# NVIDIA/retinanet-examples

Measured on AMD Instinct MI355X. Metric: images/sec end-to-end (incl. decode+NMS), RN50FPN 800px bs=8, higher is better.
Workload: dtype bf16; 1 GPU; ResNet50FPN bf16 inference, bs=8 per GPU at 800x1280, HIP decode x5 + NMS; global_batch=8, parallelism=replicas x1 (no data-path collective), entry=Model.forward (eval), postproc=fused

## Files before the change

### include/odtk_conv.h

```cpp
#ifndef ODTK_CONV_H
#define ODTK_CONV_H

#include <stddef.h>

#ifdef __cplusplus
extern "C" {
#endif

int odtk_conv_bias_act(void *y, const void *x, const void *w, const void *bias, int batch_size, int c_in, int height, int width,
                       int c_out, int kernel_h, int kernel_w, int stride_h, int stride_w, int pad_h, int pad_w, int dtype,
                       int relu, void *stream);

int odtk_conv_bias_act_pads(void *y, const void *x, const void *w, const void *bias, int batch_size, int c_in, int height, int width,
                            int c_out, int kernel_h, int kernel_w, int stride_h, int stride_w, int pad_h, int pad_w, int pad_h_end,
                            int pad_w_end, int dtype, int relu, void *stream);

const char *odtk_conv_last_plan(void);

size_t odtk_conv_plan_export(char *text, size_t capacity);
int odtk_conv_plan_import(const char *text);


int odtk_conv_instance_count(int dtype);

#ifdef __cplusplus
}
#endif
#endif
```

### include/odtk_hip.h

```cpp
#ifndef ODTK_HIP_H
#define ODTK_HIP_H

#include <stddef.h>
#include <stdint.h>

#ifdef __cplusplus
extern "C" {
#endif

#define ODTK_OK                0
#define ODTK_ERR_INVALID      -1
#define ODTK_ERR_WORKSPACE    -2
#define ODTK_ERR_HIP          -3
#define ODTK_ERR_UNSUPPORTED  -4

#define ODTK_MAX_LEVELS    6
#define ODTK_MAX_ANCHORS   32
#define ODTK_MAX_TOP_N     16384
#define ODTK_MAX_NMS_COUNT 7680
#define ODTK_MAX_NMS_COUNT_SCRATCH (1 << 22)
#define ODTK_MAX_NMS_DETECTIONS 2048

#define ODTK_F32   0
#define ODTK_BF16  1
#define ODTK_F16   2

#define ODTK_FLAG_ROTATED        1u
#define ODTK_FLAG_LOGITS         2u
#define ODTK_FLAG_ROTATED_NMS_FIXED_ANGLE 4u

const char *odtk_version(void);
int odtk_abi_struct_size(int which);
const char *odtk_last_hip_error(void);

int odtk_decode(int batch_size, const void *const *inputs, void *const *outputs,
                size_t height, size_t width, size_t scale, size_t num_anchors, size_t num_classes,
                const float *anchors, size_t anchors_len, float score_thresh, int top_n,
                void *workspace, size_t workspace_size, void *stream);

int odtk_decode_rotate(int batch_size, const void *const *inputs, void *const *outputs,
                       size_t height, size_t width, size_t scale, size_t num_anchors, size_t num_classes,
                       const float *anchors, size_t anchors_len, float score_thresh, int top_n,
                       void *workspace, size_t workspace_size, void *stream);

int odtk_nms(int batch_size, const void *const *inputs, void *const *outputs,
             size_t count, int detections_per_im, float nms_thresh,
             void *workspace, size_t workspace_size, void *stream);

int odtk_nms_rotate(int batch_size, const void *const *inputs, void *const *outputs,
                    size_t count, int detections_per_im, float nms_thresh,
                    void *workspace, size_t workspace_size, void *stream);

int odtk_iou(const void *const *inputs, void *const *outputs, int num_boxes, int num_anchors,
             void *stream);


typedef struct odtk_level {
  const void *cls;
  const void *box;
  int32_t height, width;
  int32_t stride;
  int32_t channels_last;
  const float *anchors;
  const float *cls_bias;
  const float *box_bias;
  const float *cls_thresholds;
} odtk_level_t;

#define ODTK_THRESHOLD_TABLE_FLOATS(channels) ((size_t)(channels) + 8)
int odtk_prefilter_thresholds(const float *cls_bias, int channels, int dtype, float score_thresh, float *table, void *stream);

int odtk_decode_levels(int batch_size, int n_levels, const odtk_level_t *levels,
                       int num_anchors, int num_classes, int dtype, uint32_t flags,
                       float score_thresh, int top_n,
                       void *const *outputs, int n_outputs,
                       void *workspace, size_t workspace_size, void *stream);

int odtk_nms_ex(int batch_size, const void *const *inputs, void *const *outputs, int n_outputs,
                size_t count, int detections_per_im, float nms_thresh, uint32_t flags,
                void *workspace, size_t workspace_size, void *stream);

int odtk_nms_sorted_runs(int batch_size, const void *const *inputs, void *const *outputs, int n_outputs, size_t count,
                         int run_len, const uint32_t *run_valid, int detections_per_im, float nms_thresh, uint32_t flags,
                         void *workspace, size_t workspace_size, void *stream);

int odtk_detect(int batch_size, int n_levels, const odtk_level_t *levels,
                int num_anchors, int num_classes, int dtype, uint32_t flags,
                float score_thresh, int top_n, float nms_thresh, int detections_per_im,
                void *const *outputs, void *workspace, size_t workspace_size, void *stream);

int odtk_bias_act(void *y, const float *bias, const void *residual, size_t n_pixels, int channels,
                  int dtype, int relu, void *stream);

int odtk_bias_act_maxpool(const void *y, const float *bias, void *out, int batch_size, int height, int width,
                          int channels, int dtype, int relu, void *stream);

int odtk_upsample_nearest2x(const void *x, void *out, int batch_size, int height, int width, int channels, int dtype,
                            void *stream);

int odtk_stem_pack(const void *x, void *out, int batch_size, int height, int width, int in_dtype, int channels_last, int out_dtype,
                   void *stream);

typedef struct odtk_image {
  uint64_t src_offset;
  int32_t src_width, src_height, src_pitch;
  int32_t out_width, out_height;
  int32_t mirror;
  int32_t x_table, y_table;
  int32_t x_taps, y_taps;
} odtk_image_t;
int odtk_preprocess_images(int batch_size, const odtk_image_t *images, const void *src, size_t src_bytes, const int32_t *tables,
                           size_t tables_len, const void *norm_table, void *out, int height, int width, int dtype, void *stream);

int odtk_gemm_init(const char *hipblaslt_path);
size_t odtk_gemm_plan_export(char *text, size_t capacity);
int odtk_gemm_plan_import(const char *text);
int odtk_gemm_plan_pin_misses(void);
int odtk_gemm_bias_act(void *y, const void *x, const void *w, const float *bias, const void *residual,
                       size_t m, int n, int k, int dtype, int relu,
                       void *workspace, size_t workspace_size, void *stream);

int odtk_snap_to_anchors(int batch_size, const float *targets, int n_max, const float *anchors,
                         int num_anchors, int num_classes, int height, int width, int stride,
                         float iou_background, float iou_foreground,
                         float *cls_target, float *box_target, float *depth, void *stream);

typedef struct odtk_snap_level {
  const float *anchors;
  float *cls_target;
  float *box_target;
  float *depth;
  int32_t height, width, stride, pad_;
} odtk_snap_level_t;
int odtk_snap_to_anchors_levels(int batch_size, const float *targets, int n_max, int n_levels,
                                const odtk_snap_level_t *levels, int num_anchors, int num_classes,
                                float iou_background, float iou_foreground, void *stream);

typedef struct odtk_snap_rot_level {
  const float *anchors_axis;
  const float *anchors_quads;
  float *cls_target;
  float *box_target;
  float *depth;
  int32_t height, width, stride, pad_;
} odtk_snap_rot_level_t;
int odtk_snap_to_anchors_rotated_levels(int batch_size, const float *gt_axis, const float *gt_quads, const float *gt_class,
                                        int n_max, int n_levels, const odtk_snap_rot_level_t *levels, int num_anchors,
                                        int num_classes, float iou_background, float iou_foreground, void *stream);

int odtk_retina_loss_forward(const void *cls, const void *box, const float *depth, const float *box_target,
                             int batch_size, int num_anchors, int num_classes, int height, int width,
                             int box_params, int dtype, int channels_last, float alpha, float gamma, float beta,
                             double *sums, void *stream);
int odtk_retina_loss_backward(const void *cls, const void *box, const float *depth, const float *box_target,
                              int batch_size, int num_anchors, int num_classes, int height, int width,
                              int box_params, int dtype, int channels_last, float alpha, float gamma, float beta,
                              const float *grad_cls_sum, const float *grad_box_sum, void *dcls, void *dbox,
                              void *stream);

typedef struct odtk_loss_level {
  const void *cls;
  const void *box;
  const float *depth;
  const float *box_target;
  void *dcls, *dbox;
  int32_t height, width;
  int32_t channels_last;
  int32_t pad_;
} odtk_loss_level_t;

int odtk_retina_loss_levels_forward(int n_levels, const odtk_loss_level_t *levels, int batch_size, int num_anchors,
                                    int num_classes, int box_params, int dtype, float alpha, float gamma, float beta,
                                    double *sums, void *stream);
int odtk_retina_loss_levels_forward_ws(int n_levels, const odtk_loss_level_t *levels, int batch_size, int num_anchors,
                                       int num_classes, int box_params, int dtype, float alpha, float gamma, float beta,
                                       double *sums, void *workspace, size_t workspace_size, void *stream);
int odtk_retina_loss_levels_backward(int n_levels, const odtk_loss_level_t *levels, int batch_size, int num_anchors,
                                     int num_classes, int box_params, int dtype, float alpha, float gamma, float beta,
                                     const float *grad_cls_sums, const float *grad_box_sums, void *stream);

#define ODTK_KERNEL_PREFILTER 0
#define ODTK_KERNEL_SELECT    1
#define ODTK_KERNEL_NMS       2
#define ODTK_KERNEL_IOU       3
#define ODTK_KERNEL_EPILOGUE  4
#define ODTK_KERNEL_TARGETS   5
#define ODTK_KERNEL_GEMM      6
#define ODTK_KERNEL_LOSS      7
#define ODTK_KERNEL_SELHIST   8
#define ODTK_KERNEL_SELFILTER 9
#define ODTK_KERNEL_NMS_ORDER 10
#define ODTK_KERNEL_NMS_MATRIX 11
#define ODTK_KERNEL_POOL      12
#define ODTK_KERNEL_UPSAMPLE  13
#define ODTK_KERNEL_STEM_PACK 14
#define ODTK_KERNEL_LOSS_REDUCE 15
#define ODTK_KERNEL_COUNT     16
int odtk_profile_enable(int on);
int odtk_debug_set_trace(void *device_buffer);
int odtk_debug_loss_tuning(int which, int fp32_heads, int threads, int blocks_per_cu, int unroll, int box_blocks);
int odtk_debug_loss_layout(int which, int fp32_heads, int per_wave, int window, int box_rows);
#define ODTK_LOSS_FORM_DEFAULT 1
int odtk_debug_loss_form(int form);
int odtk_profile_collect(double total_ms[ODTK_KERNEL_COUNT], int launches[ODTK_KERNEL_COUNT]);

#ifdef __cplusplus
}
#endif
#endif
```

### retinanet-examples_amd/csrc/conv_ck.cpp

```cpp
#include <hip/hip_runtime.h>

#include <array>
#include <cfloat>
#include <cstdio>
#include <cstring>
#include <map>
#include <memory>
#include <mutex>
#include <string>
#include <tuple>
#include <vector>

#include "ck/ck.hpp"
#include "ck/library/tensor_operation_instance/gpu/grouped_convolution_forward_bias_clamp.hpp"
#include "ck/tensor_operation/gpu/device/tensor_layout.hpp"
#include "ck/tensor_operation/gpu/element/element_wise_operation.hpp"

#include "../../include/odtk_conv.h"
#include "../../include/odtk_hip.h"

namespace {

using ck::index_t;
using PassThrough = ck::tensor_operation::element_wise::PassThrough;
using AddClamp = ck::tensor_operation::element_wise::AddClamp;
namespace layout = ck::tensor_layout::convolution;

template <typename T>
using ConvOp = ck::tensor_operation::device::DeviceGroupedConvFwdMultipleABD<
    2, layout::NHWGC, layout::GKYXC, ck::Tuple<layout::NHWGK>, layout::NHWGK, T, T, ck::Tuple<T>, T, PassThrough, PassThrough,
    AddClamp, T, T>;

struct Problem {
  int n, c, h, w, k, r, s, u, v, ph, pw, ph1, pw1, dtype;
  bool operator<(const Problem &o) const {
    return std::tie(n, c, h, w, k, r, s, u, v, ph, pw, ph1, pw1, dtype) <
           std::tie(o.n, o.c, o.h, o.w, o.k, o.r, o.s, o.u, o.v, o.ph, o.pw, o.ph1, o.pw1, o.dtype);
  }
};

struct Plan {
  int index = -1;
  float us = 0.0f;
  bool timed = false;
  std::string name;
};

std::mutex g_mutex;
thread_local std::string g_last_plan;

template <typename T>
struct Instances {
  std::vector<std::unique_ptr<ConvOp<T>>> ops;
  std::map<Problem, Plan> plans;
  Instances() { ops = ck::tensor_operation::device::instance::DeviceOperationInstanceFactory<ConvOp<T>>::GetInstances(); }
};

template <typename T>
Instances<T> &instances() {
  static Instances<T> inst;
  return inst;
}

template <typename T>
std::unique_ptr<ck::tensor_operation::device::BaseArgument> make_argument(ConvOp<T> &op, const Problem &p, void *y, const void *x,
                                                                          const void *w, const void *bias, int relu) {
  const index_t G = 1, N = p.n, C = p.c, K = p.k, Hi = p.h, Wi = p.w, Y = p.r, X = p.s;
  const index_t Ho = (Hi + p.ph + p.ph1 - Y) / p.u + 1, Wo = (Wi + p.pw + p.pw1 - X) / p.v + 1;
  const std::array<index_t, 5> a_len{G, N, C, Hi, Wi}, a_str{C, Hi * Wi * G * C, 1, Wi * G * C, G * C};
  const std::array<index_t, 5> b_len{G, K, C, Y, X}, b_str{K * Y * X * C, Y * X * C, 1, X * C, C};
  const std::array<index_t, 5> e_len{G, N, K, Ho, Wo}, e_str{K, Ho * Wo * G * K, 1, Wo * G * K, G * K};
  const std::array<index_t, 5> d_str{K, 0, 1, 0, 0};
  const std::array<index_t, 2> strides{p.u, p.v}, dilations{1, 1}, pads{p.ph, p.pw}, pads_end{p.ph1, p.pw1};
  return op.MakeArgumentPointer(x, w, std::array<const void *, 1>{bias}, y, a_len, a_str, b_len, b_str,
                                std::array<std::array<index_t, 5>, 1>{e_len}, std::array<std::array<index_t, 5>, 1>{d_str}, e_len,
                                e_str, strides, dilations, pads, pads_end, PassThrough{}, PassThrough{},
                                relu ? AddClamp{0.0f, FLT_MAX} : AddClamp{-FLT_MAX, FLT_MAX});
}

bool stream_is_capturing(hipStream_t stream) {
  hipStreamCaptureStatus st = hipStreamCaptureStatusNone;
  if (hipStreamIsCapturing(stream, &st) != hipSuccess) { (void)hipGetLastError(); return false; }
  return st != hipStreamCaptureStatusNone;
}

template <typename T>
bool adopt_sibling(Instances<T> &inst, const Problem &p, void *y, const void *x, const void *w, const void *bias, int relu, Plan *out) {
  const double pixels = static_cast<double>(p.n) * p.h * p.w;
  const Plan *best = nullptr;
  double best_ratio = 2.0;
  for (const auto &kv : inst.plans) {
    const Problem &q = kv.first;
    if (kv.second.index < 0 || !kv.second.timed) continue;
    if (std::tie(q.c, q.k, q.r, q.s, q.u, q.v, q.ph, q.pw, q.ph1, q.pw1, q.dtype) !=
        std::tie(p.c, p.k, p.r, p.s, p.u, p.v, p.ph, p.pw, p.ph1, p.pw1, p.dtype))
      continue;
    const double other = static_cast<double>(q.n) * q.h * q.w;
    const double ratio = other > pixels ? other / pixels : pixels / other;
    if (ratio <= best_ratio) { best_ratio = ratio; best = &kv.second; }
  }
  if (!best) return false;
  auto &op = *inst.ops[best->index];
  auto arg = make_argument<T>(op, p, y, x, w, bias, relu);
  if (!op.IsSupportedArgument(arg.get()) || op.GetWorkSpaceSize(arg.get()) != 0) return false;
  *out = *best;
  out->us = 0.0f;
  return true;
}

template <typename T>
int run(const Problem &p, void *y, const void *x, const void *w, const void *bias, int relu, hipStream_t stream, int force_index) {
  std::lock_guard<std::mutex> lock(g_mutex);
  Instances<T> &inst = instances<T>();
  Plan plan;
  auto it = inst.plans.find(p);
  if (it != inst.plans.end()) plan = it->second;
  const bool capturing = stream_is_capturing(stream);
  if (force_index >= 0) {
    plan = Plan{};
    if (force_index < static_cast<int>(inst.ops.size())) {
      auto arg = make_argument<T>(*inst.ops[force_index], p, y, x, w, bias, relu);
      if (inst.ops[force_index]->IsSupportedArgument(arg.get()) && inst.ops[force_index]->GetWorkSpaceSize(arg.get()) == 0)
        plan.index = force_index;
    }
    if (plan.index < 0) return ODTK_ERR_UNSUPPORTED;
    plan.name = inst.ops[plan.index]->GetTypeString();
  } else if (it == inst.plans.end() && adopt_sibling<T>(inst, p, y, x, w, bias, relu, &plan)) {
    inst.plans[p] = plan;
  } else if (it == inst.plans.end() || (!plan.timed && !capturing && plan.index >= 0)) {
    plan = Plan{};
    struct Events {
      hipEvent_t e0 = nullptr, e1 = nullptr;
      ~Events() {
        if (e0) (void)hipEventDestroy(e0);
        if (e1) (void)hipEventDestroy(e1);
      }
    } ev;
    if (!capturing && (hipEventCreate(&ev.e0) != hipSuccess || hipEventCreate(&ev.e1) != hipSuccess)) return ODTK_ERR_HIP;
    float best = 0.0f;
    for (size_t i = 0; i < inst.ops.size(); ++i) {
      try {
        auto &op = *inst.ops[i];
        auto arg = make_argument<T>(op, p, y, x, w, bias, relu);
        if (!op.IsSupportedArgument(arg.get()) || op.GetWorkSpaceSize(arg.get()) != 0) continue;
        if (capturing) { plan.index = static_cast<int>(i); break; }
        auto invoker = op.MakeInvokerPointer();
        const StreamConfig cfg{stream, false};
        invoker->Run(arg.get(), cfg);
        if (hipEventRecord(ev.e0, stream) != hipSuccess) { (void)hipGetLastError(); continue; }
        for (int rep = 0; rep < 3; ++rep) invoker->Run(arg.get(), cfg);
        if (hipEventRecord(ev.e1, stream) != hipSuccess) { (void)hipGetLastError(); continue; }
        if (hipEventSynchronize(ev.e1) != hipSuccess) { (void)hipGetLastError(); continue; }
        float ms = 0.0f;
        if (hipEventElapsedTime(&ms, ev.e0, ev.e1) != hipSuccess || !(ms > 0.0f)) { (void)hipGetLastError(); continue; }
        if (plan.index < 0 || ms < best) { best = ms; plan.index = static_cast<int>(i); }
      } catch (...) {
        continue;
      }
    }
    if (plan.index >= 0) {
      plan.us = best * 1000.0f / 3.0f;
      plan.timed = !capturing;
      plan.name = inst.ops[plan.index]->GetTypeString();
    } else if (!capturing) {
      plan.timed = true;
    }
    inst.plans[p] = plan;
  }
  if (plan.index < 0) return ODTK_ERR_UNSUPPORTED;
  auto &op = *inst.ops[plan.index];
  auto arg = make_argument<T>(op, p, y, x, w, bias, relu);
  op.MakeInvokerPointer()->Run(arg.get(), StreamConfig{stream, false});
  char buf[64];
  std::snprintf(buf, sizeof buf, "#%d %.1f us ", plan.index, plan.us);
  g_last_plan = std::string(buf) + plan.name;
  return hipGetLastError() == hipSuccess ? ODTK_OK : ODTK_ERR_HIP;
}

}

namespace {
template <typename T>
void export_plans(std::string *out) {
  for (const auto &kv : instances<T>().plans) {
    const Problem &p = kv.first;
    if (kv.second.index < 0 || !kv.second.timed) continue;
    char line[256];
    std::snprintf(line, sizeof line, "conv %d %d %d %d %d %d %d %d %d %d %d %d %d %d %d ", p.dtype, p.n, p.c, p.h, p.w, p.k, p.r, p.s, p.u, p.v,
                  p.ph, p.pw, p.ph1, p.pw1, kv.second.index);
    *out += line + kv.second.name + "\n";
  }
}
template <typename T>
bool import_plan(const Problem &p, int index, const std::string &name) {
  Instances<T> &inst = instances<T>();
  if (index < 0 || index >= static_cast<int>(inst.ops.size())) return false;
  if (inst.ops[index]->GetTypeString() != name) return false;
  Plan plan;
  plan.index = index;
  plan.timed = true;
  plan.name = name;
  inst.plans[p] = plan;
  return true;
}
}

extern "C" {

int odtk_conv_bias_act_pads(void *y, const void *x, const void *w, const void *bias, int batch_size, int c_in, int height, int width,
                            int c_out, int kernel_h, int kernel_w, int stride_h, int stride_w, int pad_h, int pad_w, int pad_h_end,
                            int pad_w_end, int dtype, int relu, void *stream) {
  if (!y || !x || !w || !bias || batch_size <= 0 || c_in <= 0 || c_out <= 0 || height <= 0 || width <= 0 || kernel_h <= 0 ||
      kernel_w <= 0 || stride_h <= 0 || stride_w <= 0 || pad_h < 0 || pad_w < 0 || pad_h_end < 0 || pad_w_end < 0)
    return ODTK_ERR_INVALID;
  if (height + pad_h + pad_h_end < kernel_h || width + pad_w + pad_w_end < kernel_w) return ODTK_ERR_INVALID;
  const Problem p{batch_size, c_in, height, width, c_out, kernel_h, kernel_w, stride_h, stride_w, pad_h, pad_w, pad_h_end, pad_w_end, dtype};
  int force = -1;
  if (const char *f = std::getenv("ODTK_CONV_INSTANCE")) force = std::atoi(f);
  try {
    if (dtype == ODTK_BF16) return run<ck::bhalf_t>(p, y, x, w, bias, relu, static_cast<hipStream_t>(stream), force);
    if (dtype == ODTK_F16) return run<ck::half_t>(p, y, x, w, bias, relu, static_cast<hipStream_t>(stream), force);
  } catch (const std::exception &e) {
    g_last_plan = std::string("exception: ") + e.what();
    return ODTK_ERR_UNSUPPORTED;
  } catch (...) {
    g_last_plan = "exception";
    return ODTK_ERR_UNSUPPORTED;
  }
  return ODTK_ERR_UNSUPPORTED;
}

int odtk_conv_bias_act(void *y, const void *x, const void *w, const void *bias, int batch_size, int c_in, int height, int width,
                       int c_out, int kernel_h, int kernel_w, int stride_h, int stride_w, int pad_h, int pad_w, int dtype,
                       int relu, void *stream) {
  return odtk_conv_bias_act_pads(y, x, w, bias, batch_size, c_in, height, width, c_out, kernel_h, kernel_w, stride_h, stride_w, pad_h,
                                 pad_w, pad_h, pad_w, dtype, relu, stream);
}

const char *odtk_conv_last_plan(void) { return g_last_plan.c_str(); }

size_t odtk_conv_plan_export(char *text, size_t capacity) {
  std::string out;
  try {
    std::lock_guard<std::mutex> lock(g_mutex);
    export_plans<ck::bhalf_t>(&out);
    export_plans<ck::half_t>(&out);
  } catch (...) {
    out.clear();
  }
  if (text && capacity) {
    const size_t n = out.size() < capacity - 1 ? out.size() : capacity - 1;
    std::memcpy(text, out.data(), n);
    text[n] = 0;
  }
  return out.size() + 1;
}

int odtk_conv_plan_import(const char *text) {
  if (!text) return 0;
  int taken = 0;
  try {
    std::lock_guard<std::mutex> lock(g_mutex);
    for (const char *q = text; *q;) {
      Problem p{};
      int index = -1, used = 0;
      if (std::sscanf(q, "conv %d %d %d %d %d %d %d %d %d %d %d %d %d %d %d %n", &p.dtype, &p.n, &p.c, &p.h, &p.w, &p.k, &p.r, &p.s, &p.u,
                      &p.v, &p.ph, &p.pw, &p.ph1, &p.pw1, &index, &used) == 15 && used > 0) {
        const char *name = q + used, *end = std::strchr(name, '\n');
        const std::string nm = end ? std::string(name, end) : std::string(name);
        if (p.dtype == ODTK_BF16 ? import_plan<ck::bhalf_t>(p, index, nm) : (p.dtype == ODTK_F16 && import_plan<ck::half_t>(p, index, nm)))
          ++taken;
      }
      const char *nl = std::strchr(q, '\n');
      if (!nl) break;
      q = nl + 1;
    }
  } catch (...) {
  }
  return taken;
}

int odtk_conv_instance_count(int dtype) {
  try {
    if (dtype == ODTK_BF16) return static_cast<int>(instances<ck::bhalf_t>().ops.size());
    if (dtype == ODTK_F16) return static_cast<int>(instances<ck::half_t>().ops.size());
  } catch (...) {
  }
  return 0;
}

}
```

### retinanet-examples_amd/csrc/epilogue.hpp

```cpp
#pragma once

#include "common.hpp"
#include "fastdiv.hpp"
#include "prefilter.hpp"

namespace odtk {

template <typename T>
__device__ __forceinline__ uint32_t float_to_storage(float f) {
  if constexpr (std::is_same_v<T, BF16>) return __float_as_uint(round_to_bf16(f)) >> 16;
  else return static_cast<uint32_t>(__builtin_bit_cast(uint16_t, static_cast<_Float16>(f)));
}

template <typename T, bool kResidual, bool kRelu>
__device__ __forceinline__ vuint4 bias_act_vec(vuint4 v, vuint4 r, const float *b) {
  constexpr int kPer = T::kPerLoad;
  float f[kPer];
#pragma unroll
  for (int e = 0; e < kPer; ++e) {
    float x, s = 0.0f;
    if constexpr (std::is_same_v<T, F32>) {
      x = __uint_as_float(v[e]);
      if (kResidual) s = __uint_as_float(r[e]);
    } else {
      const uint32_t hx = (v[e >> 1] >> (16 * (e & 1))) & 0xffffu, hr = (r[e >> 1] >> (16 * (e & 1))) & 0xffffu;
      x = std::is_same_v<T, BF16> ? bf16_bits_to_float(hx) : f16_bits_to_float(hx);
      if (kResidual) s = std::is_same_v<T, BF16> ? bf16_bits_to_float(hr) : f16_bits_to_float(hr);
    }
    float o = x + b[e];
    if (kResidual) o += s;
    if (kRelu) o = o > 0.0f ? o : (o != o ? o : 0.0f);
    f[e] = o;
  }
  if constexpr (std::is_same_v<T, F32>) {
#pragma unroll
    for (int e = 0; e < kPer; ++e) v[e] = __float_as_uint(f[e]);
  } else {
#pragma unroll
    for (int e = 0; e < kPer; e += 2) v[e >> 1] = float_to_storage<T>(f[e]) | (float_to_storage<T>(f[e + 1]) << 16);
  }
  return v;
}

template <typename T, bool kResidual, bool kRelu>
__global__ __launch_bounds__(256) void bias_act_kernel(void *y, const float *__restrict__ bias, const void *res,
                                                       uint64_t n_vec, uint32_t vec_per_row) {
  constexpr int kPer = T::kPerLoad;
  constexpr int kUnroll = 4;
  vuint4 *yv = static_cast<vuint4 *>(y);
  const vuint4 *rv = static_cast<const vuint4 *>(res);
  const uint64_t step = static_cast<uint64_t>(gridDim.x) * blockDim.x;
  const uint64_t q0 = static_cast<uint64_t>(blockIdx.x) * blockDim.x + threadIdx.x;
  float b[kPer];
  {
    const uint32_t c0 = static_cast<uint32_t>(q0 % vec_per_row) * kPer;
#pragma unroll
    for (int e = 0; e < kPer; ++e) b[e] = bias[c0 + e];
  }
  uint64_t q = q0;
  for (; q + (kUnroll - 1) * step < n_vec; q += kUnroll * step) {
    vuint4 v[kUnroll], r[kUnroll];
#pragma unroll
    for (int u = 0; u < kUnroll; ++u) {
      v[u] = yv[q + u * step];
      r[u] = kResidual ? rv[q + u * step] : vuint4{0, 0, 0, 0};
    }
#pragma unroll
    for (int u = 0; u < kUnroll; ++u) yv[q + u * step] = bias_act_vec<T, kResidual, kRelu>(v[u], r[u], b);
  }
  for (; q < n_vec; q += step)
    yv[q] = bias_act_vec<T, kResidual, kRelu>(yv[q], kResidual ? rv[q] : vuint4{0, 0, 0, 0}, b);
}

template <typename T, bool kResidual, bool kRelu>
__global__ void bias_act_scalar_kernel(void *y, const float *bias, const void *res, uint64_t begin, uint64_t n,
                                       uint32_t channels) {
  const uint64_t step = static_cast<uint64_t>(gridDim.x) * blockDim.x;
  for (uint64_t i = begin + static_cast<uint64_t>(blockIdx.x) * blockDim.x + threadIdx.x; i < n; i += step) {
    float o = load_raw<T>(y, i) + bias[i % channels];
    if (kResidual) o += load_raw<T>(res, i);
    if (kRelu) o = o > 0.0f ? o : (o != o ? o : 0.0f);
    if constexpr (std::is_same_v<T, F32>) static_cast<float *>(y)[i] = o;
    else static_cast<uint16_t *>(y)[i] = static_cast<uint16_t>(float_to_storage<T>(o));
  }
}

typedef short pk_short2 __attribute__((ext_vector_type(2)));
__device__ __forceinline__ uint32_t order_keys16(uint32_t w) {
  const pk_short2 sign = __builtin_bit_cast(pk_short2, w) >> 15;
  return w ^ (__builtin_bit_cast(uint32_t, sign) & 0x7fff7fffu);
}
__device__ __forceinline__ uint32_t pk_max_i16(uint32_t a, uint32_t b) {
  return __builtin_bit_cast(uint32_t, __builtin_elementwise_max(__builtin_bit_cast(pk_short2, a), __builtin_bit_cast(pk_short2, b)));
}
__device__ __forceinline__ uint32_t pk_min_i16(uint32_t a, uint32_t b) {
  return __builtin_bit_cast(uint32_t, __builtin_elementwise_min(__builtin_bit_cast(pk_short2, a), __builtin_bit_cast(pk_short2, b)));
}

struct PoolDivisors {
  FastDiv groups, wo, ho;
};

template <typename T, bool kRelu, bool k32>
__global__ __launch_bounds__(256) void bias_act_maxpool_kernel(const uint16_t *__restrict__ y, const float *__restrict__ bias,
                                                               uint16_t *__restrict__ out, uint32_t batch, uint32_t h,
                                                               uint32_t w, uint32_t c, uint32_t ho, uint32_t wo,
                                                               const PoolDivisors dv) {
  constexpr int kPer = T::kPerLoad;
  const uint32_t groups = c / kPer;
  const uint64_t total = static_cast<uint64_t>(batch) * ho * wo * groups;
  for (uint64_t i = blockIdx.x * 256ull + threadIdx.x; i < total; i += static_cast<uint64_t>(gridDim.x) * 256ull) {
    uint32_t g, ox, oy, b;
    if constexpr (k32) {
      uint32_t p = fastdivmod(static_cast<uint32_t>(i), dv.groups, &g);
      p = fastdivmod(p, dv.wo, &ox);
      b = fastdivmod(p, dv.ho, &oy);
    } else {
      g = static_cast<uint32_t>(i % groups);
      uint64_t p = i / groups;
      ox = static_cast<uint32_t>(p % wo);
      p /= wo;
      oy = static_cast<uint32_t>(p % ho);
      b = static_cast<uint32_t>(p / ho);
    }
    uint32_t kmax[4], kmin[4];
#pragma unroll
    for (int d = 0; d < 4; ++d) { kmax[d] = 0x80008000u; kmin[d] = 0x7fff7fffu; }
    const int y0 = static_cast<int>(oy) * 2 - 1, x0 = static_cast<int>(ox) * 2 - 1;
    const uint16_t *img = y + static_cast<uint64_t>(b) * h * w * c + g * kPer;
    uint32_t ro[3], co[3];
#pragma unroll
    for (int d = 0; d < 3; ++d) {
      const int yy = y0 + d < 0 ? 0 : (y0 + d >= static_cast<int>(h) ? static_cast<int>(h) - 1 : y0 + d);
      const int xx = x0 + d < 0 ? 0 : (x0 + d >= static_cast<int>(w) ? static_cast<int>(w) - 1 : x0 + d);
      ro[d] = static_cast<uint32_t>(yy) * w * c;
      co[d] = static_cast<uint32_t>(xx) * c;
    }
    vuint4 v[9];
#pragma unroll
    for (int dy = 0; dy < 3; ++dy) {
#pragma unroll
      for (int dx = 0; dx < 3; ++dx) v[dy * 3 + dx] = *reinterpret_cast<const vuint4 *>(img + (ro[dy] + co[dx]));
    }
#pragma unroll
    for (int n9 = 0; n9 < 9; ++n9) {
#pragma unroll
      for (int d = 0; d < 4; ++d) {
        const uint32_t k = order_keys16(v[n9][d]);
        kmax[d] = pk_max_i16(kmax[d], k);
        kmin[d] = pk_min_i16(kmin[d], k);
      }
    }
    float m[kPer];
#pragma unroll
    for (int e = 0; e < kPer; ++e) {
      const int32_t kx = static_cast<int16_t>(kmax[e >> 1] >> (16 * (e & 1)));
      const int32_t kn = static_cast<int16_t>(kmin[e >> 1] >> (16 * (e & 1)));
      constexpr int32_t kNegInfKey = std::is_same_v<T, BF16> ? -32641 : -31745;
      const int32_t kk = kn < kNegInfKey ? kn : kx;
      const uint32_t hx = static_cast<uint32_t>(kk ^ ((kk >> 15) & 0x7fff)) & 0xffffu;
      m[e] = std::is_same_v<T, BF16> ? bf16_bits_to_float(hx) : f16_bits_to_float(hx);
    }
    vuint4 o;
#pragma unroll
    for (int e = 0; e < kPer; e += 2) {
      float a0 = m[e] + bias[g * kPer + e], a1 = m[e + 1] + bias[g * kPer + e + 1];
      if (kRelu) { a0 = a0 > 0.0f ? a0 : (a0 != a0 ? a0 : 0.0f); a1 = a1 > 0.0f ? a1 : (a1 != a1 ? a1 : 0.0f); }
      o[e >> 1] = float_to_storage<T>(a0) | (float_to_storage<T>(a1) << 16);
    }
    *reinterpret_cast<vuint4 *>(out + ((static_cast<uint64_t>(b) * ho + oy) * wo + ox) * c + g * kPer) = o;
  }
}

__global__ __launch_bounds__(256) void upsample_nearest2x_kernel(const vuint4 *__restrict__ in, vuint4 *__restrict__ out, uint32_t h,
                                                                 uint32_t w, uint32_t groups, uint32_t total, const FastDiv by_groups,
                                                                 const FastDiv by_wo, const FastDiv by_ho) {
  for (uint32_t i = blockIdx.x * 256u + threadIdx.x; i < total; i += gridDim.x * 256u) {
    uint32_t g, ox, oy;
    uint32_t p = fastdivmod(i, by_groups, &g);
    p = fastdivmod(p, by_wo, &ox);
    const uint32_t b = fastdivmod(p, by_ho, &oy);
    out[i] = in[((static_cast<uint64_t>(b) * h + (oy >> 1)) * w + (ox >> 1)) * groups + g];
  }
}

template <typename TIn, typename TOut>
__global__ __launch_bounds__(256) void stem_pack_kernel(const void *x, void *out, uint32_t batch, uint32_t height, uint32_t width,
                                                        uint32_t channels_last, FastDiv by_wo, FastDiv by_howo) {
  const uint32_t ho = height / 2, wo = width / 2;
  const uint64_t total = static_cast<uint64_t>(batch) * ho * wo;
  const bool pairs = width % 2 == 0 && (reinterpret_cast<uintptr_t>(x) & 7u) == 0;
  for (uint64_t i = static_cast<uint64_t>(blockIdx.x) * blockDim.x + threadIdx.x; i < total; i += static_cast<uint64_t>(gridDim.x) * blockDim.x) {
    uint32_t rem, xo;
    const uint32_t n = fastdivmod(static_cast<uint32_t>(i), by_howo, &rem);
    const uint32_t yo = fastdivmod(rem, by_wo, &xo);
    float v[12];
    if (std::is_same_v<TIn, F32> && pairs) {
      const float *xf = static_cast<const float *>(x) + static_cast<uint64_t>(n) * 3 * height * width;
#pragma unroll
      for (int dy = 0; dy < 2; ++dy) {
        const uint32_t yy = 2 * yo + dy, xx = 2 * xo;
        if (channels_last) {
          const float2 *p = reinterpret_cast<const float2 *>(xf + (yy * width + xx) * 3u);
          const float2 a0 = p[0], a1 = p[1], a2 = p[2];
          v[(dy * 2) * 3 + 0] = a0.x; v[(dy * 2) * 3 + 1] = a0.y; v[(dy * 2) * 3 + 2] = a1.x;
          v[(dy * 2 + 1) * 3 + 0] = a1.y; v[(dy * 2 + 1) * 3 + 1] = a2.x; v[(dy * 2 + 1) * 3 + 2] = a2.y;
        } else {
#pragma unroll
          for (int c = 0; c < 3; ++c) {
            const float2 a0 = *reinterpret_cast<const float2 *>(xf + ((static_cast<uint32_t>(c) * height + yy) * width + xx));
            v[(dy * 2) * 3 + c] = a0.x;
            v[(dy * 2 + 1) * 3 + c] = a0.y;
          }
        }
      }
    } else {
#pragma unroll
      for (int dy = 0; dy < 2; ++dy) {
#pragma unroll
        for (int dx = 0; dx < 2; ++dx) {
#pragma unroll
          for (int c = 0; c < 3; ++c) {
            const uint64_t yy = 2 * yo + dy, xx = 2 * xo + dx;
            const uint64_t off = channels_last ? ((static_cast<uint64_t>(n) * height + yy) * width + xx) * 3 + c
                                               : ((static_cast<uint64_t>(n) * 3 + c) * height + yy) * width + xx;
            v[(dy * 2 + dx) * 3 + c] = load_raw<TIn>(x, off);
          }
        }
      }
    }
    vuint4 o0, o1;
#pragma unroll
    for (int e = 0; e < 4; ++e) o0[e] = float_to_storage<TOut>(v[2 * e]) | (float_to_storage<TOut>(v[2 * e + 1]) << 16);
    o1[0] = float_to_storage<TOut>(v[8]) | (float_to_storage<TOut>(v[9]) << 16);
    o1[1] = float_to_storage<TOut>(v[10]) | (float_to_storage<TOut>(v[11]) << 16);
    o1[2] = 0u;
    o1[3] = 0u;
    vuint4 *dst = reinterpret_cast<vuint4 *>(static_cast<uint16_t *>(out) + i * 16);
    dst[0] = o0;
    dst[1] = o1;
  }
}

}
```

### retinanet-examples_amd/csrc/odtk_hip.hip

```cpp
#include <hip/hip_runtime.h>
#include <hip/hip_ext.h>

#include <cmath>
#include <cstdio>
#include <cstdlib>
#include <atomic>
#include <cstring>
#include <mutex>
#include <utility>
#include <vector>

#include "../../include/odtk_hip.h"
#include "common.hpp"
#include "epilogue.hpp"
#include "iou.hpp"
#include "nms.hpp"
#include "prefilter.hpp"
#include "select_decode.hpp"
#include "targets.hpp"
#include "loss.hpp"
#include "gemm_lt.hpp"
#include "preprocess.hpp"

namespace {
// ... 739 lines not shown
      ODTK_HIP_TRY(hipEventElapsedTime(&ms, ev.start, ev.stop));
      total_ms[k] += ms;
      ++launches[k];
    }
  }
  return ODTK_OK;
}

int odtk_decode(int batch_size, const void *const *inputs, void *const *outputs, size_t height, size_t width,
                size_t scale, size_t num_anchors, size_t num_classes, const float *anchors, size_t anchors_len,
                float score_thresh, int top_n, void *workspace, size_t workspace_size, void *stream) {
  return decode_single(false, batch_size, inputs, outputs, height, width, scale, num_anchors, num_classes,
                       anchors, anchors_len, score_thresh, top_n, workspace, workspace_size, stream);
}

int odtk_decode_rotate(int batch_size, const void *const *inputs, void *const *outputs, size_t height,
                       size_t width, size_t scale, size_t num_anchors, size_t num_classes, const float *anchors,
                       size_t anchors_len, float score_thresh, int top_n, void *workspace, size_t workspace_size,
                       void *stream) {
  return decode_single(true, batch_size, inputs, outputs, height, width, scale, num_anchors, num_classes,
                       anchors, anchors_len, score_thresh, top_n, workspace, workspace_size, stream);
}

int odtk_nms(int batch_size, const void *const *inputs, void *const *outputs, size_t count,
             int detections_per_im, float nms_thresh, void *workspace, size_t workspace_size, void *stream) {
  return nms_impl(batch_size, inputs, outputs, 3, count, detections_per_im, nms_thresh, 0u, workspace,
                  workspace_size, static_cast<hipStream_t>(stream));
}

int odtk_nms_rotate(int batch_size, const void *const *inputs, void *const *outputs, size_t count,
                    int detections_per_im, float nms_thresh, void *workspace, size_t workspace_size,
                    void *stream) {
  return nms_impl(batch_size, inputs, outputs, 3, count, detections_per_im, nms_thresh, ODTK_FLAG_ROTATED,
                  workspace, workspace_size, static_cast<hipStream_t>(stream));
}

int odtk_nms_ex(int batch_size, const void *const *inputs, void *const *outputs, int n_outputs, size_t count,
                int detections_per_im, float nms_thresh, uint32_t flags, void *workspace,
                size_t workspace_size, void *stream) {
  return nms_impl(batch_size, inputs, outputs, n_outputs, count, detections_per_im, nms_thresh, flags,
                  workspace, workspace_size, static_cast<hipStream_t>(stream));
}

int odtk_nms_sorted_runs(int batch_size, const void *const *inputs, void *const *outputs, int n_outputs, size_t count,
                         int run_len, const uint32_t *run_valid, int detections_per_im, float nms_thresh, uint32_t flags,
                         void *workspace, size_t workspace_size, void *stream) {
  if (run_len <= 0 || count % static_cast<size_t>(run_len) != 0 || count / run_len > 8) return ODTK_ERR_INVALID;
  if (workspace && workspace_size && !run_valid) return ODTK_ERR_INVALID;
  return nms_impl(batch_size, inputs, outputs, n_outputs, count, detections_per_im, nms_thresh, flags, workspace, workspace_size,
                  static_cast<hipStream_t>(stream), static_cast<uint32_t>(run_len), run_valid);
}

int odtk_iou(const void *const *inputs, void *const *outputs, int num_boxes, int num_anchors, void *stream) {
  if (num_boxes < 0 || num_anchors < 0) return ODTK_ERR_INVALID;
  const long long pairs = 1ll * num_boxes * num_anchors;
  if (pairs == 0) return ODTK_OK;
  if (!inputs || !outputs || !inputs[0] || !inputs[1] || !outputs[0]) return ODTK_ERR_INVALID;
  if (pairs > 0x7fffffffll) return ODTK_ERR_INVALID;
  const int threads = 256;
  long long blocks = (pairs + threads - 1) / threads;
  if (blocks > 256 * 16) blocks = 256 * 16;
  {
    KernelTimer t(ODTK_KERNEL_IOU, static_cast<hipStream_t>(stream));
    hipLaunchKernelGGL(odtk::iou_pairs_kernel, dim3(static_cast<unsigned>(blocks)), dim3(threads), 0,
                       static_cast<hipStream_t>(stream), static_cast<const float *>(inputs[0]),
                       static_cast<const float *>(inputs[1]), static_cast<float *>(outputs[0]), num_boxes,
                       num_anchors);
  }
  ODTK_HIP_TRY(hipGetLastError());
  return ODTK_OK;
}

int odtk_snap_to_anchors(int batch_size, const float *targets, int n_max, const float *anchors, int num_anchors,
                         int num_classes, int height, int width, int stride, float iou_background,
                         float iou_foreground, float *cls_target, float *box_target, float *depth, void *stream) {
  if (batch_size <= 0 || n_max < 0 || num_anchors <= 0 || num_anchors > ODTK_MAX_ANCHORS || num_classes <= 0 ||
      height <= 0 || width <= 0)
    return ODTK_ERR_INVALID;
  if (!anchors || !box_target || !depth || (n_max > 0 && !targets)) return ODTK_ERR_INVALID;
  odtk::SnapArgs sa;
  std::memset(&sa, 0, sizeof sa);
  sa.targets = targets;
  sa.cls_target = cls_target;
  sa.box_target = box_target;
  sa.depth = depth;
  sa.n_max = n_max;
  sa.num_anchors = num_anchors;
  sa.num_classes = num_classes;
  sa.height = height;
  sa.width = width;
  sa.stride = static_cast<float>(stride);
  sa.iou_bg = iou_background;
  sa.iou_fg = iou_foreground;
  std::memcpy(sa.anchors, anchors, sizeof(float) * 4 * num_anchors);
  const long long cells = 1ll * num_anchors * height * width;
  const unsigned blocks = static_cast<unsigned>((cells + odtk::kSnapThreads - 1) / odtk::kSnapThreads);
  {
    KernelTimer t(ODTK_KERNEL_TARGETS, static_cast<hipStream_t>(stream));
    hipLaunchKernelGGL(odtk::snap_to_anchors_kernel, dim3(blocks, batch_size), dim3(odtk::kSnapThreads), 0,
                       static_cast<hipStream_t>(stream), sa);
  }
  ODTK_HIP_TRY(hipGetLastError());
  return ODTK_OK;
}

int odtk_snap_to_anchors_levels(int batch_size, const float *targets, int n_max, int n_levels,
                                const odtk_snap_level_t *levels, int num_anchors, int num_classes,
                                float iou_background, float iou_foreground, void *stream) {
  if (batch_size <= 0 || n_max < 0 || n_levels <= 0 || n_levels > ODTK_MAX_LEVELS || !levels || num_anchors <= 0 ||
      num_anchors > ODTK_MAX_ANCHORS || num_classes <= 0 || (n_max > 0 && !targets))
    return ODTK_ERR_INVALID;
  odtk::SnapLevelsArgs la;
  std::memset(&la, 0, sizeof la);
  la.n_levels = n_levels;
  unsigned total = 0;
  for (int l = 0; l < n_levels; ++l) {
    const odtk_snap_level_t &lv = levels[l];
    if (!lv.anchors || !lv.box_target || !lv.depth || lv.height <= 0 || lv.width <= 0) return ODTK_ERR_INVALID;
    odtk::SnapArgs &sa = la.lv[l];
    sa.targets = targets;
    sa.cls_target = lv.cls_target;
    sa.box_target = lv.box_target;
    sa.depth = lv.depth;
    sa.n_max = n_max;
    sa.num_anchors = num_anchors;
    sa.num_classes = num_classes;
    sa.height = lv.height;
    sa.width = lv.width;
    sa.stride = static_cast<float>(lv.stride);
    sa.iou_bg = iou_background;
    sa.iou_fg = iou_foreground;
    std::memcpy(sa.anchors, lv.anchors, sizeof(float) * 4 * num_anchors);
    la.block_begin[l] = total;
    const long long cells = 1ll * num_anchors * lv.height * lv.width;
    total += static_cast<unsigned>((cells + odtk::kSnapThreads - 1) / odtk::kSnapThreads);
  }
  for (int l = n_levels; l <= ODTK_MAX_LEVELS; ++l) la.block_begin[l] = total;
  timed_launch(ODTK_KERNEL_TARGETS, odtk::snap_to_anchors_levels_kernel, dim3(total, batch_size), dim3(odtk::kSnapThreads), 0,
               static_cast<hipStream_t>(stream), la);
  ODTK_HIP_TRY(hipGetLastError());
  return ODTK_OK;
}

int odtk_snap_to_anchors_rotated_levels(int batch_size, const float *gt_axis, const float *gt_quads, const float *gt_class,
                                        int n_max, int n_levels, const odtk_snap_rot_level_t *levels, int num_anchors,
                                        int num_classes, float iou_background, float iou_foreground, void *stream) {
  if (batch_size <= 0 || n_max < 0 || n_levels <= 0 || n_levels > ODTK_MAX_LEVELS || !levels || num_anchors <= 0 ||
      num_classes <= 0 || (n_max > 0 && (!gt_axis || !gt_quads || !gt_class)))
    return ODTK_ERR_INVALID;
  odtk::SnapRotLevelsArgs la;
  std::memset(&la, 0, sizeof la);
  la.n_levels = n_levels;
  unsigned total = 0;
  for (int l = 0; l < n_levels; ++l) {
    const odtk_snap_rot_level_t &lv = levels[l];
    if (!lv.anchors_axis || !lv.anchors_quads || !lv.box_target || !lv.depth || lv.height <= 0 || lv.width <= 0) return ODTK_ERR_INVALID;
    odtk::SnapRotArgs &sa = la.lv[l];
    sa.gt_axis = gt_axis; sa.gt_quads = gt_quads; sa.gt_class = gt_class;
    sa.anchors_axis = lv.anchors_axis; sa.anchors_rot = lv.anchors_quads;
    sa.cls_target = lv.cls_target; sa.box_target = lv.box_target; sa.depth = lv.depth;
    sa.n_max = n_max; sa.num_anchors = num_anchors; sa.num_classes = num_classes;
    sa.height = lv.height; sa.width = lv.width;
    sa.stride = static_cast<float>(lv.stride);
    sa.iou_bg = iou_background; sa.iou_fg = iou_foreground;
    la.block_begin[l] = total;
    const long long cells = 1ll * num_anchors * lv.height * lv.width;
    if (cells > 0x7fffffffll) return ODTK_ERR_INVALID;
    total += static_cast<unsigned>((cells + odtk::kSnapThreads - 1) / odtk::kSnapThreads);
  }
  for (int l = n_levels; l <= ODTK_MAX_LEVELS; ++l) la.block_begin[l] = total;
  timed_launch(ODTK_KERNEL_TARGETS, odtk::snap_to_anchors_rotated_levels_kernel, dim3(total, batch_size), dim3(odtk::kSnapThreads), 0,
               static_cast<hipStream_t>(stream), la);
  ODTK_HIP_TRY(hipGetLastError());
  return ODTK_OK;
}

int odtk_retina_loss_forward(const void *cls, const void *box, const float *depth, const float *box_target,
                             int batch_size, int num_anchors, int num_classes, int height, int width, int box_params,
                             int dtype, int channels_last, float alpha, float gamma, float beta, double *sums,
                             void *stream) {
  if (!sums) return ODTK_ERR_INVALID;
  ODTK_HIP_TRY(hipMemsetAsync(sums, 0, 3 * sizeof(double), static_cast<hipStream_t>(stream)));
  return retina_loss_launch(false, cls, box, depth, box_target, batch_size, num_anchors, num_classes, height, width,
                            box_params, dtype, channels_last, alpha, gamma, beta, sums, nullptr, nullptr, nullptr, nullptr,
                            static_cast<hipStream_t>(stream));
}

int odtk_retina_loss_backward(const void *cls, const void *box, const float *depth, const float *box_target,
                              int batch_size, int num_anchors, int num_classes, int height, int width, int box_params,
                              int dtype, int channels_last, float alpha, float gamma, float beta,
                              const float *grad_cls_sum, const float *grad_box_sum, void *dcls, void *dbox,
                              void *stream) {
  if (!dcls || !dbox) return ODTK_ERR_INVALID;
  if ((reinterpret_cast<uintptr_t>(dcls) | reinterpret_cast<uintptr_t>(dbox)) & 15u) return ODTK_ERR_INVALID;
  return retina_loss_launch(true, cls, box, depth, box_target, batch_size, num_anchors, num_classes, height, width,
                            box_params, dtype, channels_last, alpha, gamma, beta, nullptr, grad_cls_sum, grad_box_sum, dcls,
                            dbox, static_cast<hipStream_t>(stream));
}

int odtk_retina_loss_levels_forward(int n_levels, const odtk_loss_level_t *levels, int batch_size, int num_anchors,
                                    int num_classes, int box_params, int dtype, float alpha, float gamma, float beta,
                                    double *sums, void *stream) {
  if (!sums || n_levels <= 0 || n_levels > ODTK_MAX_LEVELS) return ODTK_ERR_INVALID;
  ODTK_HIP_TRY(hipMemsetAsync(sums, 0, 3 * sizeof(double) * n_levels, static_cast<hipStream_t>(stream)));
  return retina_loss_levels_launch(kLossFwd, n_levels, levels, batch_size, num_anchors, num_classes, box_params, dtype, alpha,
                                   gamma, beta, sums, nullptr, nullptr, nullptr, false, static_cast<hipStream_t>(stream));
}

int odtk_retina_loss_levels_forward_ws(int n_levels, const odtk_loss_level_t *levels, int batch_size, int num_anchors,
                                       int num_classes, int box_params, int dtype, float alpha, float gamma, float beta,
                                       double *sums, void *workspace, size_t workspace_size, void *stream) {
  if (n_levels <= 0 || n_levels > ODTK_MAX_LEVELS) return ODTK_ERR_INVALID;
  if (dtype != ODTK_F32 && dtype != ODTK_BF16 && dtype != ODTK_F16) return ODTK_ERR_UNSUPPORTED;
  const LossTuning t = loss_tuning_snapshot(dtype, kLossFwdWs);
  const int blocks = retina_loss_levels_launch(kLossFwdWs, n_levels, levels, batch_size, num_anchors, num_classes, box_params,
                                               dtype, alpha, gamma, beta, nullptr, nullptr, nullptr, nullptr, true, nullptr, &t);
  if (blocks < 0) return blocks;
  const size_t need = (static_cast<size_t>(blocks) * (t.per_wave ? t.threads / 64 : 1) * 3 * sizeof(double) + 255) & ~static_cast<size_t>(255);
  if (!workspace) return static_cast<int>(need);
  if (!sums) return ODTK_ERR_INVALID;
  if (workspace_size < need) return ODTK_ERR_WORKSPACE;
  if (reinterpret_cast<uintptr_t>(workspace) & 7u) return ODTK_ERR_INVALID;
  return retina_loss_levels_launch(kLossFwdWs, n_levels, levels, batch_size, num_anchors, num_classes, box_params, dtype, alpha,
                                   gamma, beta, sums, nullptr, nullptr, static_cast<double *>(workspace), false,
                                   static_cast<hipStream_t>(stream), &t);
}

int odtk_retina_loss_levels_backward(int n_levels, const odtk_loss_level_t *levels, int batch_size, int num_anchors,
                                     int num_classes, int box_params, int dtype, float alpha, float gamma, float beta,
                                     const float *grad_cls_sums, const float *grad_box_sums, void *stream) {
  return retina_loss_levels_launch(kLossBwd, n_levels, levels, batch_size, num_anchors, num_classes, box_params, dtype, alpha,
                                   gamma, beta, nullptr, grad_cls_sums, grad_box_sums, nullptr, false, static_cast<hipStream_t>(stream));
}

int odtk_bias_act_maxpool(const void *y, const float *bias, void *out, int batch_size, int height, int width,
                          int channels, int dtype, int relu, void *stream) {
  if (!y || !bias || !out || batch_size <= 0 || height <= 0 || width <= 0 || channels <= 0) return ODTK_ERR_INVALID;
  if (dtype != ODTK_BF16 && dtype != ODTK_F16) return ODTK_ERR_UNSUPPORTED;
  if (channels % 8 != 0) return ODTK_ERR_UNSUPPORTED;
  if ((reinterpret_cast<uintptr_t>(y) | reinterpret_cast<uintptr_t>(out)) & 15u) return ODTK_ERR_INVALID;
  if (1ull * height * width * channels >= (1ull << 32)) return ODTK_ERR_UNSUPPORTED;
  const uint32_t ho = (static_cast<uint32_t>(height) + 1) / 2, wo = (static_cast<uint32_t>(width) + 1) / 2;
  const uint64_t work = static_cast<uint64_t>(batch_size) * ho * wo * (channels / 8);
  uint64_t blocks = (work + 255) / 256;
  if (blocks > 256 * 32) blocks = 256 * 32;
  hipStream_t s = static_cast<hipStream_t>(stream);
  const uint16_t *in = static_cast<const uint16_t *>(y);
  uint16_t *o = static_cast<uint16_t *>(out);
  odtk::PoolDivisors dv;
  dv.groups = odtk::fastdiv_make(static_cast<uint32_t>(channels / 8));
  dv.wo = odtk::fastdiv_make(wo);
  dv.ho = odtk::fastdiv_make(ho);
  const bool small = work < (1ull << 32);
#define ODTK_POOL_(T, R, S)                                                                                             \
  timed_launch(ODTK_KERNEL_POOL, odtk::bias_act_maxpool_kernel<T, R, S>, dim3(static_cast<unsigned>(blocks)), dim3(256), 0, s, in, \
               bias, o, static_cast<uint32_t>(batch_size), static_cast<uint32_t>(height),                             \
               static_cast<uint32_t>(width), static_cast<uint32_t>(channels), ho, wo, dv)
#define ODTK_POOL(T, R) do { if (small) ODTK_POOL_(T, R, true); else ODTK_POOL_(T, R, false); } while (0)
  if (dtype == ODTK_BF16) { if (relu) ODTK_POOL(odtk::BF16, true); else ODTK_POOL(odtk::BF16, false); }
  else { if (relu) ODTK_POOL(odtk::F16, true); else ODTK_POOL(odtk::F16, false); }
#undef ODTK_POOL_
#undef ODTK_POOL
  ODTK_HIP_TRY(hipGetLastError());
  return ODTK_OK;
}

int odtk_prefilter_thresholds(const float *cls_bias, int channels, int dtype, float score_thresh, float *table, void *stream) {
  if (!cls_bias || !table || channels <= 0 || channels % 8 != 0) return ODTK_ERR_INVALID;
  if (dtype != ODTK_BF16 && dtype != ODTK_F16) return ODTK_ERR_UNSUPPORTED;
  if (reinterpret_cast<uintptr_t>(table) & 15u) return ODTK_ERR_INVALID;
  const float raw_thr = logit_lower_bound(score_thresh);
  const unsigned blocks = (static_cast<unsigned>(channels) + 255u) / 256u;
  hipStream_t s = static_cast<hipStream_t>(stream);
  if (dtype == ODTK_BF16)
    hipLaunchKernelGGL(odtk::prefilter_table_kernel<odtk::BF16>, dim3(blocks), dim3(256), 0, s, cls_bias, static_cast<uint32_t>(channels), raw_thr,
                       static_cast<uint32_t>(dtype), table);
  else
    hipLaunchKernelGGL(odtk::prefilter_table_kernel<odtk::F16>, dim3(blocks), dim3(256), 0, s, cls_bias, static_cast<uint32_t>(channels), raw_thr,
                       static_cast<uint32_t>(dtype), table);
  ODTK_HIP_TRY(hipGetLastError());
  return ODTK_OK;
}

int odtk_upsample_nearest2x(const void *x, void *out, int batch_size, int height, int width, int channels, int dtype,
                            void *stream) {
  if (!x || !out || batch_size <= 0 || height <= 0 || width <= 0 || channels <= 0) return ODTK_ERR_INVALID;
  if (dtype != ODTK_F32 && dtype != ODTK_BF16 && dtype != ODTK_F16) return ODTK_ERR_UNSUPPORTED;
  const unsigned long long row_bytes = 1ull * channels * (dtype == ODTK_F32 ? 4 : 2);
  if (row_bytes % 16) return ODTK_ERR_UNSUPPORTED;
  if ((reinterpret_cast<uintptr_t>(x) | reinterpret_cast<uintptr_t>(out)) & 15u) return ODTK_ERR_INVALID;
  const unsigned long long groups = row_bytes / 16;
  const unsigned long long total = 4ull * batch_size * height * width * groups;
  if (total > 0xf0000000ull) return ODTK_ERR_INVALID;
  unsigned long long blocks = (total + 256ull * 4 - 1) / (256ull * 4);
  if (blocks > 256 * 16) blocks = 256 * 16;
  timed_launch(ODTK_KERNEL_UPSAMPLE, odtk::upsample_nearest2x_kernel, dim3(static_cast<unsigned>(blocks)), dim3(256), 0,
               static_cast<hipStream_t>(stream), static_cast<const odtk::vuint4 *>(x), static_cast<odtk::vuint4 *>(out),
               static_cast<uint32_t>(height), static_cast<uint32_t>(width), static_cast<uint32_t>(groups), static_cast<uint32_t>(total),
               odtk::fastdiv_make(static_cast<uint32_t>(groups)), odtk::fastdiv_make(2u * width), odtk::fastdiv_make(2u * height));
  ODTK_HIP_TRY(hipGetLastError());
  return ODTK_OK;
}

int odtk_stem_pack(const void *x, void *out, int batch_size, int height, int width, int in_dtype, int channels_last, int out_dtype,
                   void *stream) {
  if (!x || !out || batch_size <= 0 || height <= 0 || width <= 0 || (height & 1) || (width & 1)) return ODTK_ERR_INVALID;
  if (channels_last != 0 && channels_last != 1) return ODTK_ERR_INVALID;
  if (in_dtype != ODTK_F32 && in_dtype != ODTK_BF16 && in_dtype != ODTK_F16) return ODTK_ERR_UNSUPPORTED;
  if (out_dtype != ODTK_BF16 && out_dtype != ODTK_F16) return ODTK_ERR_UNSUPPORTED;
  if (reinterpret_cast<uintptr_t>(out) & 15u) return ODTK_ERR_INVALID;
  if (1ull * batch_size * (height / 2) * (width / 2) > 0xf0000000ull) return ODTK_ERR_INVALID;
  if (3ull * height * width >= (1ull << 32)) return ODTK_ERR_INVALID;
  hipStream_t s = static_cast<hipStream_t>(stream);
  if (in_dtype == ODTK_F32) return stem_pack_launch<odtk::F32>(x, out, batch_size, height, width, channels_last, out_dtype, s);
  if (in_dtype == ODTK_BF16) return stem_pack_launch<odtk::BF16>(x, out, batch_size, height, width, channels_last, out_dtype, s);
  return stem_pack_launch<odtk::F16>(x, out, batch_size, height, width, channels_last, out_dtype, s);
}

static bool preprocess_axis_ok(int32_t table, int32_t taps, int32_t in_size, int32_t out_size, size_t tables_len) {
  if (table < 0) return table == -1 && in_size == out_size;
  if (taps <= 0) return false;
  const unsigned long long need = 1ull * static_cast<uint32_t>(out_size) * (2ull + static_cast<uint32_t>(taps));
  return need < (1ull << 31) && static_cast<unsigned long long>(table) + need <= tables_len;
}

int odtk_preprocess_images(int batch_size, const odtk_image_t *images, const void *src, size_t src_bytes, const int32_t *tables,
                           size_t tables_len, const void *norm_table, void *out, int height, int width, int dtype, void *stream) {
  if (!images || !src || !norm_table || !out || batch_size <= 0 || height <= 0 || width <= 0) return ODTK_ERR_INVALID;
  if (dtype != ODTK_F32 && dtype != ODTK_BF16 && dtype != ODTK_F16) return ODTK_ERR_UNSUPPORTED;
  const unsigned es = dtype == ODTK_F32 ? 4u : 2u;
  if ((reinterpret_cast<uintptr_t>(norm_table) | reinterpret_cast<uintptr_t>(out)) & (es - 1u)) return ODTK_ERR_INVALID;
  if (reinterpret_cast<uintptr_t>(tables) & 3u) return ODTK_ERR_INVALID;
  if (3ull * height * width >= (1ull << 31) || (height + odtk::kPreTileH - 1) / odtk::kPreTileH > 65535) return ODTK_ERR_INVALID;
  for (int b = 0; b < batch_size; ++b) {
    const odtk_image_t &im = images[b];
    if (im.src_width <= 0 || im.src_height <= 0 || im.out_width <= 0 || im.out_height <= 0) return ODTK_ERR_INVALID;
    if (im.out_width > width || im.out_height > height || (im.mirror != 0 && im.mirror != 1)) return ODTK_ERR_INVALID;
    if (im.src_pitch <= 0 || 3ll * im.src_width > im.src_pitch) return ODTK_ERR_INVALID;
    const unsigned long long extent = 1ull * (im.src_height - 1) * im.src_pitch + 3ull * im.src_width;
    if (extent >= (1ull << 31) || im.src_offset > src_bytes || extent > src_bytes - im.src_offset) return ODTK_ERR_INVALID;
    if ((im.x_table >= 0 || im.y_table >= 0) && !tables) return ODTK_ERR_INVALID;
    if (!preprocess_axis_ok(im.x_table, im.x_taps, im.src_width, im.out_width, tables_len) ||
        !preprocess_axis_ok(im.y_table, im.y_taps, im.src_height, im.out_height, tables_len))
      return ODTK_ERR_INVALID;
  }
  static_assert(sizeof(odtk::PreArgs) <= 4096, "kernel arguments travel by value");
  odtk::PreArgs args;
  args.src = static_cast<const uint8_t *>(src);
  args.tables = tables;
  args.norm = norm_table;
  args.out = out;
  args.height = height;
  args.width = width;
  args.vector_rows = ((3ull * width * es) % 16 == 0 && (reinterpret_cast<uintptr_t>(out) & 15u) == 0) ? 1 : 0;
  const dim3 tiles((width + odtk::kPreTileW - 1) / odtk::kPreTileW, (height + odtk::kPreTileH - 1) / odtk::kPreTileH);
  for (int first = 0; first < batch_size; first += odtk::kPreMaxImages) {
    const int n = batch_size - first < odtk::kPreMaxImages ? batch_size - first : odtk::kPreMaxImages;
    args.first = first;
    std::memcpy(args.images, images + first, sizeof(odtk_image_t) * n);
    if (n < odtk::kPreMaxImages) std::memset(args.images + n, 0, sizeof(odtk_image_t) * (odtk::kPreMaxImages - n));
    const dim3 grid(tiles.x, tiles.y, static_cast<unsigned>(n));
    if (es == 4)
      hipLaunchKernelGGL(odtk::preprocess_images_kernel<4>, grid, dim3(256), 0, static_cast<hipStream_t>(stream), args);
    else
      hipLaunchKernelGGL(odtk::preprocess_images_kernel<2>, grid, dim3(256), 0, static_cast<hipStream_t>(stream), args);
    ODTK_HIP_TRY(hipGetLastError());
  }
  return ODTK_OK;
}

int odtk_gemm_init(const char *hipblaslt_path) { return odtk::lt::init(hipblaslt_path); }

size_t odtk_gemm_plan_export(char *text, size_t capacity) { return odtk::lt::plan_export(text, capacity); }
int odtk_gemm_plan_import(const char *text) { return odtk::lt::plan_import(text); }
int odtk_gemm_plan_pin_misses(void) { return odtk::lt::pin_misses(); }

int odtk_gemm_bias_act(void *y, const void *x, const void *w, const float *bias, const void *residual, size_t m,
                       int n, int k, int dtype, int relu, void *workspace, size_t workspace_size, void *stream) {
  if (!y || !x || !w || !bias || n <= 0 || k <= 0 || residual == y) return ODTK_ERR_INVALID;
  if (dtype != ODTK_F32 && dtype != ODTK_BF16 && dtype != ODTK_F16) return ODTK_ERR_UNSUPPORTED;
  if ((reinterpret_cast<uintptr_t>(y) | reinterpret_cast<uintptr_t>(x) | reinterpret_cast<uintptr_t>(w) |
       reinterpret_cast<uintptr_t>(residual) | reinterpret_cast<uintptr_t>(workspace)) & 15u)
    return ODTK_ERR_INVALID;
  if (m == 0) return ODTK_OK;
  KernelTimer t(ODTK_KERNEL_GEMM, static_cast<hipStream_t>(stream));
  return odtk::lt::gemm_bias_act(y, x, w, bias, residual, m, static_cast<uint32_t>(n), static_cast<uint32_t>(k), dtype,
                                 relu, workspace, workspace_size, static_cast<hipStream_t>(stream));
}

int odtk_bias_act(void *y, const float *bias, const void *residual, size_t n_pixels, int channels, int dtype,
                  int relu, void *stream) {
  if (!y || !bias || channels <= 0) return ODTK_ERR_INVALID;
  if (dtype != ODTK_F32 && dtype != ODTK_BF16 && dtype != ODTK_F16) return ODTK_ERR_UNSUPPORTED;
  if ((reinterpret_cast<uintptr_t>(y) & 15u) || (reinterpret_cast<uintptr_t>(residual) & 15u)) return ODTK_ERR_INVALID;
  const uint64_t n = static_cast<uint64_t>(n_pixels) * channels;
  if (n == 0) return ODTK_OK;
  return bias_act_dispatch(y, bias, residual, n, static_cast<uint32_t>(channels), dtype, relu != 0,
                           static_cast<hipStream_t>(stream));
}

int odtk_decode_levels(int batch_size, int n_levels, const odtk_level_t *levels, int num_anchors,
                       int num_classes, int dtype, uint32_t flags, float score_thresh, int top_n,
                       void *const *outputs, int n_outputs, void *workspace, size_t workspace_size,
                       void *stream) {
  return decode_levels_impl(batch_size, n_levels, levels, num_anchors, num_classes, dtype, flags,
                            score_thresh, top_n, outputs, n_outputs, workspace, workspace_size,
                            static_cast<hipStream_t>(stream));
}

int odtk_detect(int batch_size, int n_levels, const odtk_level_t *levels, int num_anchors, int num_classes,
                int dtype, uint32_t flags, float score_thresh, int top_n, float nms_thresh,
                int detections_per_im, void *const *outputs, void *workspace, size_t workspace_size,
                void *stream) {
  if (batch_size <= 0 || n_levels <= 0 || n_levels > ODTK_MAX_LEVELS || top_n <= 0) return ODTK_ERR_INVALID;
  const int nb = (flags & ODTK_FLAG_ROTATED) ? 6 : 4;
  const size_t count = static_cast<size_t>(n_levels) * top_n;
  const int dec = decode_levels_impl(batch_size, n_levels, levels, num_anchors, num_classes, dtype, flags,
                                     score_thresh, top_n, nullptr, 0, nullptr, 0, nullptr);
  if (dec < 0) return dec;
  const int nms_ws = nms_impl(batch_size, nullptr, nullptr, 3, count, detections_per_im, nms_thresh, flags, nullptr, 0, nullptr);
  if (nms_ws < 0) return nms_ws;
  const size_t off_s = align_up(static_cast<size_t>(dec));
  const size_t off_b = off_s + align_up(sizeof(float) * batch_size * count);
  const size_t off_c = off_b + align_up(sizeof(float) * batch_size * count * nb);
  const size_t off_n = off_c + align_up(sizeof(float) * batch_size * count);
  const size_t off_v = off_n + align_up(static_cast<size_t>(nms_ws));
  const size_t total = off_v + align_up(sizeof(uint32_t) * batch_size * n_levels);
  if (!workspace || !workspace_size) return total > 0x7fffffffull ? ODTK_ERR_INVALID : static_cast<int>(total);
  if (workspace_size < total) return ODTK_ERR_WORKSPACE;
  if (!outputs) return ODTK_ERR_INVALID;
  char *ws = static_cast<char *>(workspace);
  void *cat[3] = {ws + off_s, ws + off_b, ws + off_c};
  uint32_t *run_valid = reinterpret_cast<uint32_t *>(ws + off_v);
  int rc = decode_levels_impl(batch_size, n_levels, levels, num_anchors, num_classes, dtype, flags, score_thresh,
                              top_n, cat, 3, workspace, static_cast<size_t>(dec), static_cast<hipStream_t>(stream), run_valid);
  if (rc != ODTK_OK) return rc;
  return nms_impl(batch_size, cat, outputs, 3, count, detections_per_im, nms_thresh, flags, ws + off_n,
                  static_cast<size_t>(nms_ws), static_cast<hipStream_t>(stream), static_cast<uint32_t>(top_n), run_valid);
}

}
```

### retinanet-examples_amd/odtk/_C.py

```python
import ctypes
import threading
import os

import torch

_LIB_PATH = os.environ.get('ODTK_HIP_LIBRARY') or os.path.join(os.path.dirname(os.path.abspath(__file__)), 'libodtk_hip.so')

OK, ERR_INVALID, ERR_WORKSPACE, ERR_HIP, ERR_UNSUPPORTED = 0, -1, -2, -3, -4
F32, BF16, F16 = 0, 1, 2
FLAG_ROTATED, FLAG_LOGITS, FLAG_ROTATED_NMS_FIXED_ANGLE = 1, 2, 4
MAX_LEVELS, MAX_ANCHORS, MAX_TOP_N, MAX_NMS_COUNT, MAX_NMS_COUNT_SCRATCH = 6, 32, 16384, 7680, 1 << 22

_vp = ctypes.c_void_p
_vpp = ctypes.POINTER(ctypes.c_void_p)
_fp = ctypes.POINTER(ctypes.c_float)
_sz = ctypes.c_size_t


class LossLevel(ctypes.Structure):
    _fields_ = [('cls', ctypes.c_void_p), ('box', ctypes.c_void_p), ('depth', ctypes.c_void_p), ('box_target', ctypes.c_void_p),
                ('dcls', ctypes.c_void_p), ('dbox', ctypes.c_void_p), ('height', ctypes.c_int32), ('width', ctypes.c_int32),
                ('channels_last', ctypes.c_int32), ('pad_', ctypes.c_int32)]


class SnapLevel(ctypes.Structure):
    _fields_ = [('anchors', ctypes.POINTER(ctypes.c_float)), ('cls_target', ctypes.c_void_p), ('box_target', ctypes.c_void_p),
                ('depth', ctypes.c_void_p), ('height', ctypes.c_int32), ('width', ctypes.c_int32), ('stride', ctypes.c_int32),
                ('pad_', ctypes.c_int32)]


class SnapRotLevel(ctypes.Structure):
    _fields_ = [('anchors_axis', ctypes.c_void_p), ('anchors_quads', ctypes.c_void_p), ('cls_target', ctypes.c_void_p),
                ('box_target', ctypes.c_void_p), ('depth', ctypes.c_void_p), ('height', ctypes.c_int32), ('width', ctypes.c_int32),
                ('stride', ctypes.c_int32), ('pad_', ctypes.c_int32)]


class Level(ctypes.Structure):
    _fields_ = [('cls', _vp), ('box', _vp), ('height', ctypes.c_int32), ('width', ctypes.c_int32),
                ('stride', ctypes.c_int32), ('channels_last', ctypes.c_int32), ('anchors', _fp),
                ('cls_bias', _vp), ('box_bias', _vp), ('cls_thresholds', _vp)]


class Image(ctypes.Structure):
    _fields_ = [('src_offset', ctypes.c_uint64), ('src_width', ctypes.c_int32), ('src_height', ctypes.c_int32),
                ('src_pitch', ctypes.c_int32), ('out_width', ctypes.c_int32), ('out_height', ctypes.c_int32),
                ('mirror', ctypes.c_int32), ('x_table', ctypes.c_int32), ('y_table', ctypes.c_int32),
                ('x_taps', ctypes.c_int32), ('y_taps', ctypes.c_int32)]


_SIGNATURES = {
    'odtk_version': (ctypes.c_char_p, []),
    'odtk_abi_struct_size': (ctypes.c_int, [ctypes.c_int]),
    'odtk_last_hip_error': (ctypes.c_char_p, []),
    'odtk_decode': (ctypes.c_int, [ctypes.c_int, _vpp, _vpp, _sz, _sz, _sz, _sz, _sz, _fp, _sz, ctypes.c_float,
                                   ctypes.c_int, _vp, _sz, _vp]),
    'odtk_decode_rotate': (ctypes.c_int, [ctypes.c_int, _vpp, _vpp, _sz, _sz, _sz, _sz, _sz, _fp, _sz,
                                          ctypes.c_float, ctypes.c_int, _vp, _sz, _vp]),
    'odtk_nms': (ctypes.c_int, [ctypes.c_int, _vpp, _vpp, _sz, ctypes.c_int, ctypes.c_float, _vp, _sz, _vp]),
    'odtk_nms_rotate': (ctypes.c_int, [ctypes.c_int, _vpp, _vpp, _sz, ctypes.c_int, ctypes.c_float, _vp, _sz, _vp]),
    'odtk_iou': (ctypes.c_int, [_vpp, _vpp, ctypes.c_int, ctypes.c_int, _vp]),
    'odtk_decode_levels': (ctypes.c_int, [ctypes.c_int, ctypes.c_int, ctypes.POINTER(Level), ctypes.c_int,
                                          ctypes.c_int, ctypes.c_int, ctypes.c_uint32, ctypes.c_float, ctypes.c_int,
                                          _vpp, ctypes.c_int, _vp, _sz, _vp]),
    'odtk_nms_ex': (ctypes.c_int, [ctypes.c_int, _vpp, _vpp, ctypes.c_int, _sz, ctypes.c_int, ctypes.c_float,
                                   ctypes.c_uint32, _vp, _sz, _vp]),
    'odtk_detect': (ctypes.c_int, [ctypes.c_int, ctypes.c_int, ctypes.POINTER(Level), ctypes.c_int, ctypes.c_int,
                                   ctypes.c_int, ctypes.c_uint32, ctypes.c_float, ctypes.c_int, ctypes.c_float,
                                   ctypes.c_int, _vpp, _vp, _sz, _vp]),
    'odtk_snap_to_anchors': (ctypes.c_int, [ctypes.c_int, _vp, ctypes.c_int, _fp, ctypes.c_int, ctypes.c_int,
                                            ctypes.c_int, ctypes.c_int, ctypes.c_int, ctypes.c_float, ctypes.c_float,
                                            _vp, _vp, _vp, _vp]),
    'odtk_snap_to_anchors_levels': (ctypes.c_int, [ctypes.c_int, _vp, ctypes.c_int, ctypes.c_int, ctypes.POINTER(SnapLevel),
                                                   ctypes.c_int, ctypes.c_int, ctypes.c_float, ctypes.c_float, _vp]),
    'odtk_retina_loss_forward': (ctypes.c_int, [_vp, _vp, _vp, _vp] + [ctypes.c_int] * 8 + [ctypes.c_float] * 3 + [_vp, _vp]),
    'odtk_retina_loss_backward': (ctypes.c_int, [_vp, _vp, _vp, _vp] + [ctypes.c_int] * 8 + [ctypes.c_float] * 3 +
                                  [_vp, _vp, _vp, _vp, _vp]),
    'odtk_retina_loss_levels_forward': (ctypes.c_int, [ctypes.c_int, ctypes.POINTER(LossLevel)] + [ctypes.c_int] * 5 +
                                        [ctypes.c_float] * 3 + [_vp, _vp]),
    'odtk_retina_loss_levels_forward_ws': (ctypes.c_int, [ctypes.c_int, ctypes.POINTER(LossLevel)] + [ctypes.c_int] * 5 +
                                           [ctypes.c_float] * 3 + [_vp, _vp, _sz, _vp]),
    'odtk_retina_loss_levels_backward': (ctypes.c_int, [ctypes.c_int, ctypes.POINTER(LossLevel)] + [ctypes.c_int] * 5 +
                                         [ctypes.c_float] * 3 + [_vp, _vp, _vp]),
    'odtk_bias_act': (ctypes.c_int, [_vp, _vp, _vp, _sz, ctypes.c_int, ctypes.c_int, ctypes.c_int, _vp]),
    'odtk_profile_enable': (ctypes.c_int, [ctypes.c_int]),
    'odtk_debug_set_trace': (ctypes.c_int, [_vp]),
    'odtk_debug_loss_tuning': (ctypes.c_int, [ctypes.c_int] * 6),
    'odtk_debug_loss_layout': (ctypes.c_int, [ctypes.c_int] * 5),
    'odtk_debug_loss_form': (ctypes.c_int, [ctypes.c_int]),
    'odtk_bias_act_maxpool': (ctypes.c_int, [ctypes.c_void_p, ctypes.c_void_p, ctypes.c_void_p, ctypes.c_int, ctypes.c_int,
                                             ctypes.c_int, ctypes.c_int, ctypes.c_int, ctypes.c_int, ctypes.c_void_p]),
    'odtk_snap_to_anchors_rotated_levels': (ctypes.c_int, [ctypes.c_int, _vp, _vp, _vp, ctypes.c_int, ctypes.c_int,
                                                           ctypes.POINTER(SnapRotLevel), ctypes.c_int, ctypes.c_int, ctypes.c_float,
                                                           ctypes.c_float, _vp]),
    'odtk_prefilter_thresholds': (ctypes.c_int, [_vp, ctypes.c_int, ctypes.c_int, ctypes.c_float, _vp, _vp]),
    'odtk_upsample_nearest2x': (ctypes.c_int, [ctypes.c_void_p, ctypes.c_void_p, ctypes.c_int, ctypes.c_int, ctypes.c_int, ctypes.c_int,
                                               ctypes.c_int, ctypes.c_void_p]),
    'odtk_stem_pack': (ctypes.c_int, [ctypes.c_void_p, ctypes.c_void_p, ctypes.c_int, ctypes.c_int, ctypes.c_int, ctypes.c_int,
                                      ctypes.c_int, ctypes.c_int, ctypes.c_void_p]),
    'odtk_preprocess_images': (ctypes.c_int, [ctypes.c_int, ctypes.POINTER(Image), _vp, _sz, _vp, _sz, _vp, _vp, ctypes.c_int, ctypes.c_int,
                                              ctypes.c_int, _vp]),
    'odtk_nms_sorted_runs': (ctypes.c_int, [ctypes.c_int, _vpp, _vpp, ctypes.c_int, _sz, ctypes.c_int, _vp, ctypes.c_int, ctypes.c_float,
                                            ctypes.c_uint32, _vp, _sz, _vp]),
    'odtk_gemm_init': (ctypes.c_int, [ctypes.c_char_p]),
    'odtk_gemm_plan_export': (ctypes.c_size_t, [ctypes.c_char_p, ctypes.c_size_t]),
    'odtk_gemm_plan_import': (ctypes.c_int, [ctypes.c_char_p]),
    'odtk_gemm_plan_pin_misses': (ctypes.c_int, []),
    'odtk_gemm_bias_act': (ctypes.c_int, [ctypes.c_void_p, ctypes.c_void_p, ctypes.c_void_p, ctypes.c_void_p, ctypes.c_void_p,
                                          ctypes.c_size_t, ctypes.c_int, ctypes.c_int, ctypes.c_int, ctypes.c_int,
                                          ctypes.c_void_p, ctypes.c_size_t, ctypes.c_void_p]),
    'odtk_profile_collect': (ctypes.c_int, [ctypes.POINTER(ctypes.c_double), ctypes.POINTER(ctypes.c_int)]),
}

KERNEL_NAMES = ('prefilter_scan_kernel', 'select_decode_kernel', 'nms_kernel', 'iou_pairs_kernel', 'bias_act_kernel',
                'snap_to_anchors_kernel', 'gemm_bias_act', 'retina_loss_kernel', 'select_hist_kernel', 'select_filter_kernel',
                'nms_first_round_kernel', 'rotated_sup_matrix_kernel', 'bias_act_maxpool_kernel', 'upsample_nearest2x_kernel',
                'stem_pack_kernel', 'loss_reduce_kernel')
traffic_count = False
traffic_bytes = {}


def _count(name, nbytes):
    if traffic_count:
        traffic_bytes[name] = traffic_bytes.get(name, 0) + int(nbytes)


_lib = None


def library():
    global _lib
    if _lib is None:
        if not os.path.isfile(_LIB_PATH):
            raise ImportError('odtk._C: %s is missing -- build the HIP library first '
                              '(python __graft_entry__.py, or make -C retinanet-examples_amd/csrc). '
                              'There is no CPU fallback.' % _LIB_PATH)
        lib = ctypes.CDLL(_LIB_PATH)
        for name, (res, args) in _SIGNATURES.items():
            fn = getattr(lib, name)
            fn.restype = res
            fn.argtypes = args
        for which, mirror in ((0, Level), (1, SnapLevel), (2, SnapRotLevel), (3, LossLevel), (5, Image)):
            if lib.odtk_abi_struct_size(which) != ctypes.sizeof(mirror):
                raise ImportError('odtk._C: %s was built from another revision of include/odtk_hip.h (sizeof struct %d: library %d, '
                                  'binding %d) -- rebuild it (make -C retinanet-examples_amd/csrc)'
                                  % (_LIB_PATH, which, lib.odtk_abi_struct_size(which), ctypes.sizeof(mirror)))
        _lib = lib
        for part in filter(None, os.environ.get('ODTK_LOSS_TUNING', '').split(';')):
            side, _, vals = part.partition(':')
            side = side.strip()
            _check(lib.odtk_debug_loss_tuning({'fwd': 0, 'bwd': 1, 'ws': 2}[side[:-2]], int(side.endswith('32')),
                                              *(int(v) for v in vals.split(','))), 'ODTK_LOSS_TUNING')
        if os.environ.get('ODTK_LOSS_FORM', '') != '':
            import warnings
            warnings.warn('odtk._C: ODTK_LOSS_FORM=%s overrides the loss kernels\' arithmetic form for this process' % os.environ['ODTK_LOSS_FORM'])
            _check(lib.odtk_debug_loss_form(int(os.environ['ODTK_LOSS_FORM'])), 'ODTK_LOSS_FORM')
    return _lib


def exported_symbols():
    return [n for n in _SIGNATURES]


_ERR = {ERR_INVALID: 'invalid argument', ERR_WORKSPACE: 'Workspace is too small!',
        ERR_HIP: 'HIP error', ERR_UNSUPPORTED: 'unsupported dtype/layout'}


def _check(rc, what):
    if rc < 0:
        detail = library().odtk_last_hip_error().decode() if rc == ERR_HIP else ''
        raise RuntimeError('%s failed: %s%s' % (what, _ERR.get(rc, 'error %d' % rc), (' (%s)' % detail) if detail else ''))
    return rc


def _check_input(t, name):
    if not isinstance(t, torch.Tensor) or not t.is_cuda:
        raise RuntimeError('%s must be a CUDA tensor' % name)
    if not t.is_contiguous():
        raise RuntimeError('%s must be contiguous' % name)
    if t.dtype != torch.float32:
        raise RuntimeError('%s must be float32' % name)


def _ptrs(tensors):
    return (ctypes.c_void_p * len(tensors))(*[t.data_ptr() if t is not None else None for t in tensors])


_workspaces = {}
_workspaces_lock = threading.Lock()


def _workspace(device, nbytes):
    stream = torch.cuda.current_stream(device)
    if torch.cuda.is_current_stream_capturing():
        return torch.empty(max(nbytes, 256), dtype=torch.uint8, device=device), stream.cuda_stream
    key = (device.index, stream.cuda_stream)
    with _workspaces_lock:
        ws = _workspaces.get(key)
        if ws is None or ws.numel() < nbytes:
            ws = torch.empty(max(nbytes, 256), dtype=torch.uint8, device=device)
            _workspaces[key] = ws
    return ws, stream.cuda_stream


def _anchor_array(anchors):
    flat = [float(v) for v in anchors]
    return (ctypes.c_float * len(flat))(*flat), len(flat)


def decode(cls_head, box_head, anchors, scale, score_thresh, top_n, rotated=False):
    _check_input(cls_head, 'cls_head')
    _check_input(box_head, 'box_head')
    lib = library()
    nb = 6 if rotated else 4
    batch, channels, height, width = cls_head.shape
    arr, n = _anchor_array(anchors)
    num_anchors = n // 4
    if num_anchors == 0 or n % 4 or channels % num_anchors:
        raise RuntimeError('decode: %d anchor values do not describe the %d channels of cls_head' % (n, channels))
    num_classes = channels // num_anchors
    if box_head.shape != (batch, num_anchors * nb, height, width):
        raise RuntimeError('box_head shape %s does not match cls_head %s' % (tuple(box_head.shape), tuple(cls_head.shape)))
    fn = lib.odtk_decode_rotate if rotated else lib.odtk_decode
    with torch.cuda.device(cls_head.device):
        scores = torch.empty((batch, top_n), dtype=torch.float32, device=cls_head.device)
        boxes = torch.empty((batch, top_n, nb), dtype=torch.float32, device=cls_head.device)
        classes = torch.empty((batch, top_n), dtype=torch.float32, device=cls_head.device)
        size = _check(fn(batch, None, None, height, width, int(scale), num_anchors, num_classes, arr, n,
                         float(score_thresh), int(top_n), None, 0, None), 'decode (workspace query)')
        ws, stream = _workspace(cls_head.device, size)
        _check(fn(batch, _ptrs([cls_head, box_head]), _ptrs([scores, boxes, classes]), height, width, int(scale),
                  num_anchors, num_classes, arr, n, float(score_thresh), int(top_n), ws.data_ptr(), ws.numel(),
                  stream), 'decode')
    return [scores, boxes, classes]


def nms(scores, boxes, classes, nms_thresh, detections_per_im, rotated=False, return_indices=False):
    _check_input(scores, 'scores')
    _check_input(boxes, 'boxes')
    _check_input(classes, 'classes')
    lib = library()
    nb = 6 if rotated else 4
    batch, count = scores.shape
    if boxes.shape != (batch, count, nb) or classes.shape != (batch, count):
        raise RuntimeError('nms: inconsistent shapes')
    dev = scores.device
    with torch.cuda.device(dev):
        out = [torch.empty((batch, detections_per_im), dtype=torch.float32, device=dev),
               torch.empty((batch, detections_per_im, nb), dtype=torch.float32, device=dev),
               torch.empty((batch, detections_per_im), dtype=torch.float32, device=dev)]
        if return_indices:
            out.append(torch.empty((batch, detections_per_im), dtype=torch.int32, device=dev))
        flags = FLAG_ROTATED if rotated else 0
        size = _check(lib.odtk_nms_ex(batch, None, None, len(out), count, int(detections_per_im), float(nms_thresh),
                                      flags, None, 0, None), 'nms (workspace query)')
        ws, stream = _workspace(dev, size)
        _check(lib.odtk_nms_ex(batch, _ptrs([scores, boxes, classes]), _ptrs(out), len(out), count,
                               int(detections_per_im), float(nms_thresh), flags, ws.data_ptr(), ws.numel(), stream),
               'nms')
    return out


def nms_sorted_runs(scores, boxes, classes, run_len, nms_thresh, detections_per_im, rotated=False):
    _check_input(scores, 'scores')
    _check_input(boxes, 'boxes')
    _check_input(classes, 'classes')
    lib = library()
    nb = 6 if rotated else 4
    batch, count = scores.shape
    if boxes.shape != (batch, count, nb) or classes.shape != (batch, count) or count % int(run_len):
        raise RuntimeError('nms_sorted_runs: inconsistent shapes')
    dev = scores.device
    with torch.cuda.device(dev):
        run_valid = (scores.view(batch, count // int(run_len), int(run_len)) > 0).sum(2).to(torch.int32).contiguous()
        out = [torch.empty((batch, detections_per_im), dtype=torch.float32, device=dev),
               torch.empty((batch, detections_per_im, nb), dtype=torch.float32, device=dev),
               torch.empty((batch, detections_per_im), dtype=torch.float32, device=dev)]
        flags = FLAG_ROTATED if rotated else 0
        size = _check(lib.odtk_nms_sorted_runs(batch, None, None, 3, count, int(run_len), None, int(detections_per_im),
                                               float(nms_thresh), flags, None, 0, None), 'nms_sorted_runs (workspace query)')
        ws, stream = _workspace(dev, size)
        _check(lib.odtk_nms_sorted_runs(batch, _ptrs([scores, boxes, classes]), _ptrs(out), 3, count, int(run_len),
                                        run_valid.data_ptr(), int(detections_per_im), float(nms_thresh), flags, ws.data_ptr(),
                                        ws.numel(), stream), 'nms_sorted_runs')
    return out


def iou(boxes, anchors):
    _check_input(boxes, 'boxes')
    _check_input(anchors, 'anchors')
    lib = library()
    num_boxes = boxes.numel() // 8
    num_anchors = anchors.numel() // 8
    with torch.cuda.device(boxes.device):
        out = torch.empty((num_anchors, num_boxes), dtype=torch.float32, device=boxes.device)
        stream = torch.cuda.current_stream(boxes.device).cuda_stream
        _check(lib.odtk_iou(_ptrs([boxes, anchors]), _ptrs([out]), num_boxes, num_anchors, stream), 'iou')
    return [out]


_DTYPES = {torch.float32: F32, torch.bfloat16: BF16, torch.float16: F16}


def _pair_layout(c, b, cname, bname, what, prefer_channels_last=False):
    def readings(t, name):
        if not isinstance(t, torch.Tensor) or not t.is_cuda:
            raise RuntimeError('%s must be a CUDA tensor' % name)
        if t.dim() != 4:
            raise RuntimeError('%s must be 4-d [B, C, H, W]' % name)
        n, l = t.is_contiguous(), t.is_contiguous(memory_format=torch.channels_last)
        if not (n or l):
            raise RuntimeError('%s must be contiguous (NCHW or channels_last)' % name)
        return n, l
    cn, cl = readings(c, cname)
    bn, bl = readings(b, bname)
    if prefer_channels_last and cl and bl:
        return 1
    if cn and bn:
        return 0
    if cl and bl:
        return 1
    raise RuntimeError('%s%s and %s must share one memory format' % (what, cname, bname))


def prefilter_thresholds(cls_bias, dtype, score_thresh):
    if not cls_bias.is_cuda or cls_bias.dtype != torch.float32 or not cls_bias.is_contiguous() or cls_bias.numel() % 8:
        raise RuntimeError('prefilter_thresholds: cls_bias must be a contiguous float32 CUDA vector whose length is a multiple of 8')
    if dtype not in (torch.bfloat16, torch.float16):
        raise RuntimeError('prefilter_thresholds: 16-bit head dtypes only')
    table = torch.empty(cls_bias.numel() + 8, dtype=torch.float32, device=cls_bias.device)
    with torch.cuda.device(cls_bias.device):
        stream = torch.cuda.current_stream(cls_bias.device).cuda_stream
        _check(library().odtk_prefilter_thresholds(cls_bias.data_ptr(), cls_bias.numel(), _DTYPES[dtype], float(score_thresh),
                                                   table.data_ptr(), stream), 'prefilter_thresholds')
    return table


def _levels(cls_heads, box_heads, anchors_list, strides, nb, cls_bias=None, box_bias=None, cls_thresholds=None):
    n = len(cls_heads)
    if not (n == len(box_heads) == len(anchors_list) == len(strides)) or n == 0 or n > MAX_LEVELS:
        raise RuntimeError('decode_levels: need 1..%d levels with matching lists' % MAX_LEVELS)
    batch = cls_heads[0].shape[0]
    dtype = cls_heads[0].dtype
    if dtype not in _DTYPES:
        raise RuntimeError('decode_levels: unsupported dtype %s' % dtype)
    arr = (Level * n)()
    keep = []
    num_anchors = None
    for i, (c, b, a, s) in enumerate(zip(cls_heads, box_heads, anchors_list, strides)):
        lay = _pair_layout(c, b, 'cls_head[%d]' % i, 'box_head[%d]' % i, '', prefer_channels_last=cls_bias is not None)
        if c.dtype != dtype or b.dtype != dtype:
            raise RuntimeError('decode_levels: all head tensors must share one dtype')
        flat = a.reshape(-1).tolist() if isinstance(a, torch.Tensor) else list(a)
        carr, ln = _anchor_array(flat)
        keep.append(carr)
        if num_anchors is None:
            num_anchors = ln // 4
        if ln != 4 * num_anchors or c.shape[0] != batch or b.shape != (batch, num_anchors * nb, c.shape[2], c.shape[3]):
            raise RuntimeError('decode_levels: inconsistent level %d' % i)
        arr[i].cls = c.data_ptr()
        arr[i].box = b.data_ptr()
        arr[i].height, arr[i].width = c.shape[2], c.shape[3]
        arr[i].stride = int(s)
        arr[i].channels_last = lay
        arr[i].anchors = ctypes.cast(carr, _fp)
        for name, bias, width in (('cls_bias', cls_bias, c.shape[1]), ('box_bias', box_bias, b.shape[1]),
                                  ('cls_thresholds', cls_thresholds if cls_bias is not None else None, c.shape[1] + 8)):
            if bias is None:
                continue
            t = bias[i] if isinstance(bias, (list, tuple)) else bias
            if t is None:
                continue
            if not t.is_cuda or t.dtype != torch.float32 or t.numel() != width or not t.is_contiguous():
                raise RuntimeError('decode_levels: %s must be a contiguous float32 CUDA vector of length %d' % (name, width))
            keep.append(t)
            setattr(arr[i], name, t.data_ptr())
    num_classes = cls_heads[0].shape[1] // num_anchors
    return arr, keep, batch, num_anchors, num_classes, _DTYPES[dtype]


def decode_levels(cls_heads, box_heads, anchors_list, strides, score_thresh, top_n, rotated=False,
                  return_indices=False, logits=False, cls_bias=None, box_bias=None, cls_thresholds=None):
    lib = library()
    nb = 6 if rotated else 4
    arr, keep, batch, num_anchors, num_classes, dtype = _levels(cls_heads, box_heads, anchors_list, strides, nb,
                                                                cls_bias, box_bias, cls_thresholds)
    dev = cls_heads[0].device
    n = len(cls_heads)
    with torch.cuda.device(dev):
        out = [torch.empty((batch, n * top_n), dtype=torch.float32, device=dev),
               torch.empty((batch, n * top_n, nb), dtype=torch.float32, device=dev),
               torch.empty((batch, n * top_n), dtype=torch.float32, device=dev)]
        if return_indices:
            out.append(torch.empty((batch, n * top_n), dtype=torch.int32, device=dev))
        flags = (FLAG_ROTATED if rotated else 0) | (FLAG_LOGITS if logits else 0)
        size = _check(lib.odtk_decode_levels(batch, n, arr, num_anchors, num_classes, dtype, flags, float(score_thresh),
                                             int(top_n), None, 0, None, 0, None), 'decode_levels (workspace query)')
        ws, stream = _workspace(dev, size)
        _check(lib.odtk_decode_levels(batch, n, arr, num_anchors, num_classes, dtype, flags, float(score_thresh),
                                      int(top_n), _ptrs(out), len(out), ws.data_ptr(), ws.numel(), stream),
               'decode_levels')
    return out


def detect(cls_heads, box_heads, anchors_list, strides, score_thresh, top_n, nms_thresh, detections_per_im,
           rotated=False, logits=False, cls_bias=None, box_bias=None, cls_thresholds=None):
    lib = library()
    nb = 6 if rotated else 4
    arr, keep, batch, num_anchors, num_classes, dtype = _levels(cls_heads, box_heads, anchors_list, strides, nb,
                                                                cls_bias, box_bias, cls_thresholds)
    dev = cls_heads[0].device
    n = len(cls_heads)
    with torch.cuda.device(dev):
        out = [torch.empty((batch, detections_per_im), dtype=torch.float32, device=dev),
               torch.empty((batch, detections_per_im, nb), dtype=torch.float32, device=dev),
               torch.empty((batch, detections_per_im), dtype=torch.float32, device=dev)]
        flags = (FLAG_ROTATED if rotated else 0) | (FLAG_LOGITS if logits else 0)
        args = (batch, n, arr, num_anchors, num_classes, dtype, flags, float(score_thresh), int(top_n),
                float(nms_thresh), int(detections_per_im))
        size = _check(lib.odtk_detect(*args, None, None, 0, None), 'detect (workspace query)')
        ws, stream = _workspace(dev, size)
        _check(lib.odtk_detect(*args, _ptrs(out), ws.data_ptr(), ws.numel(), stream), 'detect')
    return out


def snap_to_anchors(targets, anchors, num_classes, height, width, stride, iou_background, iou_foreground,
                    want_cls_target=True):
    _check_input(targets, 'targets')
    if targets.dim() != 3 or targets.shape[2] != 5:
        raise RuntimeError('targets must be [B, N, 5]')
    arr, n = _anchor_array(anchors.reshape(-1).tolist() if isinstance(anchors, torch.Tensor) else anchors)
    a = n // 4
    b, n_max = targets.shape[0], targets.shape[1]
    dev = targets.device
    with torch.cuda.device(dev):
        cls = torch.empty((b, a, num_classes, height, width), dtype=torch.float32, device=dev) if want_cls_target else None
        box_t = torch.empty((b, a, 4, height, width), dtype=torch.float32, device=dev)
        depth = torch.empty((b, a, 1, height, width), dtype=torch.float32, device=dev)
        stream = torch.cuda.current_stream(dev).cuda_stream
        _check(library().odtk_snap_to_anchors(b, targets.data_ptr(), n_max, arr, a, int(num_classes), int(height),
                                              int(width), int(stride), float(iou_background), float(iou_foreground),
                                              cls.data_ptr() if cls is not None else None, box_t.data_ptr(),
                                              depth.data_ptr(), stream),
               'snap_to_anchors')
    return cls, box_t, depth


def snap_to_anchors_rotated_levels(gt_axis, gt_quads, gt_class, anchors_list, num_classes, sizes, strides, iou_background,
                                   iou_foreground, want_cls_target=True):
    for t, name, last in ((gt_axis, 'gt_axis', 6), (gt_quads, 'gt_quads', 8)):
        _check_input(t, name)
        if t.dim() != 3 or t.shape[2] != last:
            raise RuntimeError('%s must be [B, N, %d]' % (name, last))
    _check_input(gt_class, 'gt_class')
    n = len(anchors_list)
    if not (n == len(sizes) == len(strides)) or n == 0 or n > MAX_LEVELS:
        raise RuntimeError('snap_to_anchors_rotated_levels: need 1..%d levels with matching lists' % MAX_LEVELS)
    b, n_max = gt_axis.shape[0], gt_axis.shape[1]
    if gt_quads.shape[:2] != (b, n_max) or tuple(gt_class.shape) != (b, n_max):
        raise RuntimeError('snap_to_anchors_rotated_levels: gt_axis / gt_quads / gt_class disagree')
    dev = gt_axis.device
    arr = (SnapRotLevel * n)()
    cls_t, box_t, depth_t = [], [], []
    a = None
    with torch.cuda.device(dev):
        for i, ((axis, quads), (h, w), s) in enumerate(zip(anchors_list, sizes, strides)):
            _check_input(axis, 'anchors (axis form)')
            _check_input(quads, 'anchors (quads)')
            if a is None:
                a = axis.shape[0]
            if tuple(axis.shape) != (a, 4) or tuple(quads.shape) != (a, 8):
                raise RuntimeError('snap_to_anchors_rotated_levels: every level needs [A, 4] and [A, 8] anchor tables')
            cls_t.append(torch.empty((b, a, num_classes, h, w), dtype=torch.float32, device=dev) if want_cls_target else None)
            box_t.append(torch.empty((b, a, 6, h, w), dtype=torch.float32, device=dev))
            depth_t.append(torch.empty((b, a, 1, h, w), dtype=torch.float32, device=dev))
            arr[i].anchors_axis, arr[i].anchors_quads = axis.data_ptr(), quads.data_ptr()
            arr[i].cls_target = cls_t[-1].data_ptr() if want_cls_target else None
            arr[i].box_target, arr[i].depth = box_t[-1].data_ptr(), depth_t[-1].data_ptr()
            arr[i].height, arr[i].width, arr[i].stride = int(h), int(w), int(s)
        stream = torch.cuda.current_stream(dev).cuda_stream
        _check(library().odtk_snap_to_anchors_rotated_levels(b, gt_axis.data_ptr(), gt_quads.data_ptr(), gt_class.data_ptr(), n_max, n,
                                                             arr, a, int(num_classes), float(iou_background), float(iou_foreground),
                                                             stream), 'snap_to_anchors_rotated_levels')
    return cls_t, box_t, depth_t


def snap_to_anchors_levels(targets, anchors_list, num_classes, sizes, strides, iou_background, iou_foreground,
                           want_cls_target=True):
    _check_input(targets, 'targets')
    if targets.dim() != 3 or targets.shape[2] != 5:
        raise RuntimeError('targets must be [B, N, 5]')
    n = len(anchors_list)
    if not (n == len(sizes) == len(strides)) or n == 0 or n > MAX_LEVELS:
        raise RuntimeError('snap_to_anchors_levels: need 1..%d levels with matching lists' % MAX_LEVELS)
    b, n_max = targets.shape[0], targets.shape[1]
    dev = targets.device
    arr = (SnapLevel * n)()
    keep, cls_t, box_t, depth_t = [], [], [], []
    a = None
    with torch.cuda.device(dev):
        for i, (anchors, (h, w), s) in enumerate(zip(anchors_list, sizes, strides)):
            carr, ln = _anchor_array(anchors.reshape(-1).tolist() if isinstance(anchors, torch.Tensor) else anchors)
            if a is None:
                a = ln // 4
            if ln != 4 * a:
                raise RuntimeError('snap_to_anchors_levels: every level needs the same number of anchors')
            keep.append(carr)
            cls_t.append(torch.empty((b, a, num_classes, h, w), dtype=torch.float32, device=dev) if want_cls_target else None)
            box_t.append(torch.empty((b, a, 4, h, w), dtype=torch.float32, device=dev))
            depth_t.append(torch.empty((b, a, 1, h, w), dtype=torch.float32, device=dev))
            arr[i].anchors = ctypes.cast(carr, _fp)
            arr[i].cls_target = cls_t[-1].data_ptr() if want_cls_target else None
            arr[i].box_target, arr[i].depth = box_t[-1].data_ptr(), depth_t[-1].data_ptr()
            arr[i].height, arr[i].width, arr[i].stride = int(h), int(w), int(s)
        stream = torch.cuda.current_stream(dev).cuda_stream
        _check(library().odtk_snap_to_anchors_levels(b, targets.data_ptr(), n_max, n, arr, a, int(num_classes),
                                                     float(iou_background), float(iou_foreground), stream),
               'snap_to_anchors_levels')
    return cls_t, box_t, depth_t


def _loss_geometry(cls_head, box_head, depth, box_target):
    if not (cls_head.is_cuda and box_head.is_cuda and depth.is_cuda and box_target.is_cuda):
        raise RuntimeError('retina_loss: tensors must be on the GPU')
    if cls_head.dim() != 4 or box_head.dim() != 4 or depth.dim() != 5 or box_target.dim() != 5:
        raise RuntimeError('retina_loss: cls/box must be [B, ch, H, W], depth [B, A, 1, H, W], box_target [B, A, nb, H, W]')
    lay = _pair_layout(cls_head, box_head, 'cls_head', 'box_head', 'retina_loss: ')
    b, ch, h, w = cls_head.shape
    a, nb = box_target.shape[1], box_target.shape[2]
    if cls_head.dtype not in _DTYPES or box_head.dtype != cls_head.dtype:
        raise RuntimeError('retina_loss: heads must share one dtype out of float32 / bfloat16 / float16')
    if ch % a or depth.shape != (b, a, 1, h, w) or box_target.shape != (b, a, nb, h, w) or box_head.shape != (b, a * nb, h, w):
        raise RuntimeError('retina_loss: inconsistent shapes')
    if depth.dtype != torch.float32 or box_target.dtype != torch.float32 or not depth.is_contiguous() or not box_target.is_contiguous():
        raise RuntimeError('retina_loss: depth and box_target must be contiguous float32')
    return b, a, ch // a, h, w, nb, _DTYPES[cls_head.dtype], lay


def _loss_levels(cls_heads, box_heads, depths, box_targets, grads=None):
    n = len(cls_heads)
    if not (n == len(box_heads) == len(depths) == len(box_targets)) or n == 0 or n > MAX_LEVELS:
        raise RuntimeError('retina_loss_levels: need 1..%d levels with matching lists' % MAX_LEVELS)
    arr = (LossLevel * n)()
    geo = None
    for i in range(n):
        b, a, c, h, w, nb, dtype, lay = _loss_geometry(cls_heads[i], box_heads[i], depths[i], box_targets[i])
        if geo is None:
            geo = (b, a, c, nb, dtype)
        elif geo != (b, a, c, nb, dtype):
            raise RuntimeError('retina_loss_levels: every level must share batch, anchors, classes, box parameters and dtype')
        arr[i].cls, arr[i].box = cls_heads[i].data_ptr(), box_heads[i].data_ptr()
        arr[i].depth, arr[i].box_target = depths[i].data_ptr(), box_targets[i].data_ptr()
        arr[i].height, arr[i].width, arr[i].channels_last = h, w, lay
        if grads is not None:
            arr[i].dcls, arr[i].dbox = grads[0][i].data_ptr(), grads[1][i].data_ptr()
    return arr, n, geo


def retina_loss_levels_forward(cls_heads, box_heads, depths, box_targets, alpha, gamma, beta, reproducible=False):
    arr, n, (b, a, c, nb, dtype) = _loss_levels(cls_heads, box_heads, depths, box_targets)
    dev = cls_heads[0].device
    lib = library()
    with torch.cuda.device(dev):
        sums = torch.empty((n, 3), dtype=torch.float64, device=dev)
        if not reproducible:
            stream = torch.cuda.current_stream(dev).cuda_stream
            _check(lib.odtk_retina_loss_levels_forward(n, arr, b, a, c, nb, dtype, float(alpha), float(gamma), float(beta),
                                                       sums.data_ptr(), stream), 'retina_loss_levels_forward')
            return sums
        need = _check(lib.odtk_retina_loss_levels_forward_ws(n, arr, b, a, c, nb, dtype, float(alpha), float(gamma), float(beta),
                                                             None, None, 0, None), 'retina_loss_levels_forward (workspace query)')
        ws, stream = _workspace(dev, need)
        _check(lib.odtk_retina_loss_levels_forward_ws(n, arr, b, a, c, nb, dtype, float(alpha), float(gamma), float(beta),
                                                      sums.data_ptr(), ws.data_ptr(), ws.numel(), stream), 'retina_loss_levels_forward')
    return sums


def retina_loss_levels_backward(cls_heads, box_heads, depths, box_targets, alpha, gamma, beta, grad_cls_sums, grad_box_sums):
    dev = cls_heads[0].device
    with torch.cuda.device(dev):
        dcls = [torch.empty_like(t) for t in cls_heads]
        dbox = [torch.empty_like(t) for t in box_heads]
        for g, t in zip(dcls + dbox, list(cls_heads) + list(box_heads)):
            if g.stride() != t.stride():
                raise RuntimeError('retina_loss_levels_backward: could not allocate gradients in the heads\' layout')
        arr, n, (b, a, c, nb, dtype) = _loss_levels(cls_heads, box_heads, depths, box_targets, (dcls, dbox))

        def vec(g):
            return None if g is None else g.detach().to(device=dev, dtype=torch.float32).reshape(n).contiguous()

        g_cls, g_box = vec(grad_cls_sums), vec(grad_box_sums)
        stream = torch.cuda.current_stream(dev).cuda_stream
        _check(library().odtk_retina_loss_levels_backward(n, arr, b, a, c, nb, dtype, float(alpha), float(gamma), float(beta),
                                                          g_cls.data_ptr() if g_cls is not None else None,
                                                          g_box.data_ptr() if g_box is not None else None, stream),
               'retina_loss_levels_backward')
    return dcls, dbox


def retina_loss_forward(cls_head, box_head, depth, box_target, alpha, gamma, beta):
    b, a, c, h, w, nb, dtype, lay = _loss_geometry(cls_head, box_head, depth, box_target)
    dev = cls_head.device
    with torch.cuda.device(dev):
        sums = torch.empty(3, dtype=torch.float64, device=dev)
        stream = torch.cuda.current_stream(dev).cuda_stream
        _check(library().odtk_retina_loss_forward(cls_head.data_ptr(), box_head.data_ptr(), depth.data_ptr(),
                                                  box_target.data_ptr(), b, a, c, h, w, nb, dtype, lay, float(alpha),
                                                  float(gamma), float(beta), sums.data_ptr(), stream), 'retina_loss_forward')
    return sums


def retina_loss_backward(cls_head, box_head, depth, box_target, alpha, gamma, beta, grad_cls_sum, grad_box_sum):
    b, a, c, h, w, nb, dtype, lay = _loss_geometry(cls_head, box_head, depth, box_target)
    dev = cls_head.device

    def scalar(g):
        if g is None:
            return None
        g = g.detach().to(device=dev, dtype=torch.float32).reshape(1)
        return g

    g_cls, g_box = scalar(grad_cls_sum), scalar(grad_box_sum)
    with torch.cuda.device(dev):
        dcls = torch.empty_like(cls_head)
        dbox = torch.empty_like(box_head)
        if dcls.stride() != cls_head.stride() or dbox.stride() != box_head.stride():
            raise RuntimeError('retina_loss_backward: could not allocate gradients in the heads\' layout')
        stream = torch.cuda.current_stream(dev).cuda_stream
        _check(library().odtk_retina_loss_backward(cls_head.data_ptr(), box_head.data_ptr(), depth.data_ptr(),
                                                   box_target.data_ptr(), b, a, c, h, w, nb, dtype, lay, float(alpha),
                                                   float(gamma), float(beta),
                                                   g_cls.data_ptr() if g_cls is not None else None,
                                                   g_box.data_ptr() if g_box is not None else None,
                                                   dcls.data_ptr(), dbox.data_ptr(), stream), 'retina_loss_backward')
    return dcls, dbox


def bias_act_(y, bias, residual=None, relu=True):
    if not y.is_cuda or y.dim() != 4 or y.dtype not in _DTYPES:
        raise RuntimeError('bias_act_: y must be a 4-d CUDA tensor of float32/bfloat16/float16')
    n, c, h, w = y.shape
    if not (y.is_contiguous(memory_format=torch.channels_last) or h * w == 1):
        raise RuntimeError('bias_act_: y must be channels_last')
    if bias.dtype != torch.float32 or bias.numel() != c or not bias.is_cuda:
        raise RuntimeError('bias_act_: bias must be a float32 CUDA vector of length C')
    if residual is not None and (residual.shape != y.shape or residual.dtype != y.dtype or not (
            residual.is_contiguous(memory_format=torch.channels_last) or h * w == 1)):
        raise RuntimeError('bias_act_: residual must match y (shape, dtype, channels_last)')
    with torch.cuda.device(y.device):
        stream = torch.cuda.current_stream(y.device).cuda_stream
        _check(library().odtk_bias_act(y.data_ptr(), bias.data_ptr(), residual.data_ptr() if residual is not None else None,
                                       n * h * w, c, _DTYPES[y.dtype], 1 if relu else 0, stream), 'bias_act')
    _count('bias_act_kernel', y.numel() * y.element_size() * (3 if residual is not None else 2))
    return y


def bias_act_maxpool(y, bias, relu=True):
    if not y.is_cuda or y.dim() != 4 or y.dtype not in (torch.bfloat16, torch.float16):
        raise RuntimeError('bias_act_maxpool: y must be a 4-d CUDA tensor of bfloat16/float16')
    n, c, h, w = y.shape
    if not y.is_contiguous(memory_format=torch.channels_last) or c % 8:
        raise RuntimeError('bias_act_maxpool: y must be channels_last with channels % 8 == 0')
    if bias.dtype != torch.float32 or bias.numel() != c or not bias.is_cuda:
        raise RuntimeError('bias_act_maxpool: bias must be a float32 CUDA vector of length C')
    out = torch.empty((n, c, (h + 1) // 2, (w + 1) // 2), dtype=y.dtype, device=y.device, memory_format=torch.channels_last)
    with torch.cuda.device(y.device):
        stream = torch.cuda.current_stream(y.device).cuda_stream
        _check(library().odtk_bias_act_maxpool(y.data_ptr(), bias.data_ptr(), out.data_ptr(), n, h, w, c, _DTYPES[y.dtype],
                                               1 if relu else 0, stream), 'bias_act_maxpool')
    _count('bias_act_maxpool_kernel', (y.numel() + out.numel()) * y.element_size())
    return out


def upsample2x(x):
    if not x.is_cuda or x.dim() != 4 or x.dtype not in _DTYPES:
        raise RuntimeError('upsample2x: x must be a 4-d CUDA tensor of float32/bfloat16/float16')
    n, c, h, w = x.shape
    if not x.is_contiguous(memory_format=torch.channels_last) or (c * x.element_size()) % 16:
        raise RuntimeError('upsample2x: x must be channels_last with channels * element size a multiple of 16 bytes')
    out = torch.empty((n, c, 2 * h, 2 * w), dtype=x.dtype, device=x.device, memory_format=torch.channels_last)
    with torch.cuda.device(x.device):
        stream = torch.cuda.current_stream(x.device).cuda_stream
        _check(library().odtk_upsample_nearest2x(x.data_ptr(), out.data_ptr(), n, h, w, c, _DTYPES[x.dtype], stream), 'upsample2x')
    _count('upsample_nearest2x_kernel', (x.numel() + out.numel()) * x.element_size())
    return out


def stem_pack(x, dtype):
    if not x.is_cuda or x.dim() != 4 or x.shape[1] != 3 or x.dtype not in _DTYPES or dtype not in (torch.bfloat16, torch.float16):
        raise RuntimeError('stem_pack: x must be a [B, 3, H, W] CUDA tensor of float32/bfloat16/float16, dtype bfloat16/float16')
    n, _, h, w = x.shape
    if h % 2 or w % 2:
        raise RuntimeError('stem_pack: height and width must be even')
    if x.is_contiguous():
        cl = 0
    elif x.is_contiguous(memory_format=torch.channels_last):
        cl = 1
    else:
        raise RuntimeError('stem_pack: x must be contiguous (NCHW or channels_last)')
    out = torch.empty((n, 16, h // 2, w // 2), dtype=dtype, device=x.device, memory_format=torch.channels_last)
    with torch.cuda.device(x.device):
        stream = torch.cuda.current_stream(x.device).cuda_stream
        _check(library().odtk_stem_pack(x.data_ptr(), out.data_ptr(), n, h, w, _DTYPES[x.dtype], cl, _DTYPES[dtype], stream), 'stem_pack')
    return out


def preprocess_images(src, images, tables, table, height, width):
    if not src.is_cuda or src.dtype != torch.uint8 or not src.is_contiguous():
        raise RuntimeError('preprocess_images: src must be a contiguous uint8 CUDA tensor')
    if tables.device != src.device or tables.dtype != torch.int32 or not tables.is_contiguous():
        raise RuntimeError('preprocess_images: tables must be a contiguous int32 tensor on the device of src')
    if table.device != src.device or table.dtype not in _DTYPES or tuple(table.shape) != (3, 256) or not table.is_contiguous():
        raise RuntimeError('preprocess_images: table must be a contiguous [3, 256] float32/bfloat16/float16 tensor on the device of src')
    if not isinstance(images, ctypes.Array):
        images = (Image * len(images))(*images)
    batch = len(images)
    out = torch.empty((batch, 3, height, width), dtype=table.dtype, device=src.device, memory_format=torch.channels_last)
    with torch.cuda.device(src.device):
        stream = torch.cuda.current_stream(src.device).cuda_stream
        _check(library().odtk_preprocess_images(batch, images, src.data_ptr(), src.numel(), tables.data_ptr() if tables.numel() else None,
                                                tables.numel(), table.data_ptr(), out.data_ptr(), height, width, _DTYPES[table.dtype],
                                                stream), 'preprocess_images')
    return out


_GEMM_WORKSPACE = {}
_GEMM_READY = []


def _gemm_setup(device):
    if not gemm_available():
        raise RuntimeError('gemm_bias_act: hipBLASLt could not be bound (odtk_gemm_init failed)')
    if torch.cuda.is_current_stream_capturing():
        return torch.empty(32 << 20, dtype=torch.uint8, device=device)
    key = (device, torch.cuda.current_stream(device).cuda_stream)
    if key not in _GEMM_WORKSPACE:
        _GEMM_WORKSPACE[key] = torch.empty(32 << 20, dtype=torch.uint8, device=device)
    return _GEMM_WORKSPACE[key]


def gemm_available():
    if not _GEMM_READY:
        shipped = os.path.join(os.path.dirname(torch.__file__), 'lib', 'libhipblaslt.so')
        path = shipped if os.path.exists(shipped) else None
        rc = library().odtk_gemm_init(path.encode() if path else None)
        _GEMM_READY.append(rc == OK)
    return _GEMM_READY[0]


def gemm_bias_act(x, weight, bias, residual=None, relu=True):
    if not x.is_cuda or x.dim() != 4 or x.dtype not in _DTYPES:
        raise RuntimeError('gemm_bias_act: x must be a 4-d CUDA tensor of float32/bfloat16/float16')
    b, k, h, w = x.shape
    n = weight.shape[0]
    if weight.numel() != n * k or weight.dtype != x.dtype or not weight.is_contiguous() and not weight.is_contiguous(
            memory_format=torch.channels_last):
        raise RuntimeError('gemm_bias_act: weight must be a dense [Cout, Cin(, 1, 1)] tensor of x.dtype')
    if not (x.is_contiguous(memory_format=torch.channels_last) or h * w == 1):
        raise RuntimeError('gemm_bias_act: x must be channels_last')
    if bias.dtype != torch.float32 or bias.numel() != n or not bias.is_cuda:
        raise RuntimeError('gemm_bias_act: bias must be a float32 CUDA vector of length Cout')
    y = torch.empty((b, n, h, w), dtype=x.dtype, device=x.device, memory_format=torch.channels_last)
    if residual is not None and (residual.shape != y.shape or residual.dtype != y.dtype or not (
            residual.is_contiguous(memory_format=torch.channels_last) or h * w == 1)):
        raise RuntimeError('gemm_bias_act: residual must match the output (shape, dtype, channels_last)')
    with torch.cuda.device(x.device):
        ws = _gemm_setup(x.device)
        stream = torch.cuda.current_stream(x.device).cuda_stream
        _check(library().odtk_gemm_bias_act(y.data_ptr(), x.data_ptr(), weight.data_ptr(), bias.data_ptr(),
                                            residual.data_ptr() if residual is not None else None,
                                            b * h * w, n, k, _DTYPES[x.dtype], 1 if relu else 0,
                                            ws.data_ptr(), ws.numel(), stream), 'gemm_bias_act')
    return y


_CONV_LIB_PATH = os.path.join(os.path.dirname(os.path.abspath(__file__)), 'libodtk_conv.so')
_conv_lib = []


def conv_library():
    if not _conv_lib:
        lib = None
        if os.path.isfile(_CONV_LIB_PATH) and not os.environ.get('ODTK_NO_CONV_LIBRARY'):
            lib = ctypes.CDLL(_CONV_LIB_PATH)
            lib.odtk_conv_bias_act.restype = ctypes.c_int
            lib.odtk_conv_bias_act.argtypes = [ctypes.c_void_p] * 4 + [ctypes.c_int] * 13 + [ctypes.c_void_p]
            lib.odtk_conv_bias_act_pads.restype = ctypes.c_int
            lib.odtk_conv_bias_act_pads.argtypes = [ctypes.c_void_p] * 4 + [ctypes.c_int] * 15 + [ctypes.c_void_p]
            lib.odtk_conv_last_plan.restype = ctypes.c_char_p
            lib.odtk_conv_last_plan.argtypes = []
            lib.odtk_conv_instance_count.restype = ctypes.c_int
            lib.odtk_conv_instance_count.argtypes = [ctypes.c_int]
            lib.odtk_conv_plan_export.restype = ctypes.c_size_t
            lib.odtk_conv_plan_export.argtypes = [ctypes.c_char_p, ctypes.c_size_t]
            lib.odtk_conv_plan_import.restype = ctypes.c_int
            lib.odtk_conv_plan_import.argtypes = [ctypes.c_char_p]
        _conv_lib.append(lib)
    return _conv_lib[0]


def conv_available():
    return conv_library() is not None


def conv_bias_act(x, weight, bias, stride=(1, 1), padding=(1, 1), relu=True, out=None):
    lib = conv_library()
    if lib is None:
        raise ImportError('odtk._C: %s is missing -- build it (python __graft_entry__.py, or make -C retinanet-examples_amd/csrc conv)'
                          % _CONV_LIB_PATH)
    if not x.is_cuda or x.dim() != 4 or x.dtype not in (torch.bfloat16, torch.float16):
        raise RuntimeError('conv_bias_act: x must be a 4-d CUDA tensor of bfloat16/float16')
    b, c, h, w = x.shape
    k, c2, kh, kw = weight.shape
    if c2 != c or weight.dtype != x.dtype or not weight.is_contiguous(memory_format=torch.channels_last):
        raise RuntimeError('conv_bias_act: weight must be [Cout, Cin, kh, kw] of x.dtype, channels_last')
    if not x.is_contiguous(memory_format=torch.channels_last):
        raise RuntimeError('conv_bias_act: x must be channels_last')
    if bias.dtype != x.dtype or bias.numel() != k or not bias.is_cuda or not bias.is_contiguous():
        raise RuntimeError('conv_bias_act: bias must be a CUDA vector of length Cout in the dtype of x')
    sh, sw = (stride, stride) if isinstance(stride, int) else stride
    ph, pw = (padding, padding) if isinstance(padding, int) else padding
    (ph0, ph1), (pw0, pw1) = [(p, p) if isinstance(p, int) else p for p in (ph, pw)]
    ho, wo = (h + ph0 + ph1 - kh) // sh + 1, (w + pw0 + pw1 - kw) // sw + 1
    if out is None:
        y = torch.empty((b, k, ho, wo), dtype=x.dtype, device=x.device, memory_format=torch.channels_last)
    else:
        if tuple(out.shape) != (b, k, ho, wo) or out.dtype != x.dtype or out.device != x.device or \
                not out.is_contiguous(memory_format=torch.channels_last):
            raise RuntimeError('conv_bias_act: out must be a channels_last %s tensor of shape %s' % (x.dtype, (b, k, ho, wo)))
        y = out
    with torch.cuda.device(x.device):
        stream = torch.cuda.current_stream(x.device).cuda_stream
        _check(lib.odtk_conv_bias_act_pads(y.data_ptr(), x.data_ptr(), weight.data_ptr(), bias.data_ptr(), b, c, h, w, k, kh, kw,
                                           sh, sw, ph0, pw0, ph1, pw1, _DTYPES[x.dtype], 1 if relu else 0, stream), 'conv_bias_act')
    return y


def conv_last_plan():
    lib = conv_library()
    return lib.odtk_conv_last_plan().decode() if lib is not None else ''


def _export_text(fn):
    need = fn(None, 0)
    buf = ctypes.create_string_buffer(int(need))
    fn(buf, need)
    return buf.value.decode()


def library_plans_export():
    text = _export_text(library().odtk_gemm_plan_export)
    lib = conv_library()
    if lib is not None:
        text += _export_text(lib.odtk_conv_plan_export)
    return text


def library_plans_import(text):
    data = text.encode()
    gemm_available()
    n_gemm = library().odtk_gemm_plan_import(data)
    lib = conv_library()
    return n_gemm, (lib.odtk_conv_plan_import(data) if lib is not None else 0)


def gemm_plan_pin_misses():
    return library().odtk_gemm_plan_pin_misses()


def loss_tuning(which, fp32_heads, threads, blocks_per_cu, unroll, box_blocks):
    _check(library().odtk_debug_loss_tuning(int(which), int(bool(fp32_heads)), int(threads), int(blocks_per_cu),
                                            int(unroll), int(box_blocks)), 'loss_tuning')


def loss_layout(which, fp32_heads, per_wave=0, window=0, box_rows=1):
    _check(library().odtk_debug_loss_layout(int(which), int(bool(fp32_heads)), int(bool(per_wave)), int(bool(window)),
                                            int(bool(box_rows))), 'loss_layout')


LOSS_FORM_DEFAULT = 1


def loss_form(form):
    _check(library().odtk_debug_loss_form(int(form)), 'loss_form')


TRACE_WORDS = 16384


def debug_set_trace(trace):
    if trace is None:
        return library().odtk_debug_set_trace(None)
    if not (trace.is_cuda and trace.dtype == torch.int64 and trace.is_contiguous() and trace.numel() >= TRACE_WORDS):
        raise ValueError('the trace buffer must be a contiguous int64 CUDA tensor of >= %d elements (128 KiB)' % TRACE_WORDS)
    return library().odtk_debug_set_trace(trace.data_ptr())


def profile_enable(on=True, kernels=None):
    if not on:
        mask = 0
    elif kernels is None:
        mask = -1
    else:
        mask = 0
        for k in kernels:
            mask |= 1 << KERNEL_NAMES.index(k)
    _check(library().odtk_profile_enable(mask), 'profile_enable')


def profile_collect():
    ms = (ctypes.c_double * len(KERNEL_NAMES))()
    n = (ctypes.c_int * len(KERNEL_NAMES))()
    _check(library().odtk_profile_collect(ms, n), 'profile_collect')
    return {name: (ms[i], n[i]) for i, name in enumerate(KERNEL_NAMES)}


class Engine:

    def __init__(self, *args, **kwargs):
        raise NotImplementedError('odtk._C.Engine: the TensorRT engine path is not available on MI355X')

    @staticmethod
    def load(path):
        raise NotImplementedError('odtk._C.Engine.load: the TensorRT engine path is not available on MI355X')
```

### retinanet-examples_amd/odtk/fused.py

```python
import hashlib
import json
import os
import threading

import torch
import torch.nn as nn
import torch.nn.functional as F

from . import _C
from . import box as box_ops
from .backbones.resnet import BasicBlock, Bottleneck


_PLAN_LOCK = threading.Lock()
_TLS = threading.local()


def _planning():
    return getattr(_TLS, 'planning', False)


def _key_str(key):
    kind, shape = ('only', key[1:]) if key and key[0] == 'only' else ('act', key)
    return kind + ':' + 'x'.join(str(int(v)) for v in shape)


def _str_key(text):
    kind, shape = text.split(':')
    shape = tuple(int(v) for v in shape.split('x'))
    return (('only',) + shape) if kind == 'only' else shape


def fold_conv_bn(conv, bn=None):
    w = conv.weight.detach().float()
    b = conv.bias.detach().float() if conv.bias is not None else torch.zeros(w.shape[0], device=w.device)
    if bn is not None:
        eps = getattr(bn, 'eps', 1e-5)
        scale = bn.weight.detach().float() / torch.sqrt(bn.running_var.detach().float() + eps)
        w = w * scale.view(-1, 1, 1, 1)
        b = (b - bn.running_mean.detach().float()) * scale + bn.bias.detach().float()
    return w, b


def stem_space_to_depth_weights(w):
    w4 = torch.zeros(w.shape[0], 16, 4, 4, dtype=w.dtype, device=w.device)
    for dy in range(2):
        for dx in range(2):
            for r4 in range(4):
                for s4 in range(4):
                    r, s_ = 2 * r4 + dy - 1, 2 * s4 + dx - 1
                    if 0 <= r < 7 and 0 <= s_ < 7:
                        w4[:, (dy * 2 + dx) * 3:(dy * 2 + dx) * 3 + 3, r4, s4] = w[:, :, r, s_]
    return w4


def space_to_depth_pack(x):
    b, _, h, w = x.shape
    xs = x.view(b, 3, h // 2, 2, w // 2, 2).permute(0, 3, 5, 1, 2, 4).reshape(b, 12, h // 2, w // 2)
    return torch.cat([xs, torch.zeros(b, 4, h // 2, w // 2, dtype=x.dtype, device=x.device)], 1)


class _Conv(nn.Module):

    use_conv_library = True
    route_mode = os.environ.get('ODTK_CONV_ROUTE', 'auto')

    def __init__(self, conv, bn=None, relu=False, dtype=torch.bfloat16):
        super().__init__()
        w, b = fold_conv_bn(conv, bn)
        self.register_buffer('weight', w.to(dtype).contiguous(memory_format=torch.channels_last))
        self.register_buffer('bias', b.contiguous())
        self.register_buffer('bias_lp', b.to(dtype).contiguous())
        self.stride, self.padding, self.relu, self.groups = conv.stride, conv.padding, relu, conv.groups
        self.pointwise = (tuple(conv.kernel_size) == (1, 1) and tuple(conv.padding) == (0, 0) and conv.groups == 1
                          and tuple(conv.dilation) == (1, 1))
        self.library_ok = (not self.pointwise and conv.groups == 1 and tuple(conv.dilation) == (1, 1)
                           and dtype in (torch.bfloat16, torch.float16) and w.shape[1] % 8 == 0)
        self.strided_ok = (self.pointwise and tuple(conv.stride) != (1, 1) and dtype in (torch.bfloat16, torch.float16)
                           and w.shape[1] % 8 == 0)
        self.zero_bias = None
        self.learned = {}
        self.route = {}

    def conv_only(self, x, out=None):
        if (self.library_ok and _Conv.use_conv_library and x.is_cuda and x.is_contiguous(memory_format=torch.channels_last)
                and _C.conv_available()):
            key = ('only',) + tuple(x.shape)
            if self.zero_bias is None:
                self.zero_bias = torch.zeros_like(self.bias_lp)
            if self._routed(key, 'only', x, self._miopen_only, self._library_only):
                try:
                    return self._library_only(x, out)
                except RuntimeError:
                    self.route[key] = (False, float('inf'), 0.0)
        y = self._miopen_only(x)
        return y if out is None else out.copy_(y)

    def _miopen_only(self, x):
        y = F.conv2d(x, self.weight, None, self.stride, self.padding, groups=self.groups)
        return y if y.is_contiguous(memory_format=torch.channels_last) else y.contiguous(memory_format=torch.channels_last)

    def _library_only(self, x, out=None):
        return _C.conv_bias_act(x, self.weight, self.zero_bias, self.stride, self.padding, False, out=out)

    def _two_pass(self, x, residual=None):
        y = F.conv2d(x, self.weight, None, self.stride, self.padding, groups=self.groups)
        if not y.is_contiguous(memory_format=torch.channels_last):
            y = y.contiguous(memory_format=torch.channels_last)
        return _C.bias_act_(y, self.bias, residual, self.relu)

    def _copy_then_gemm(self, x, residual=None):
        x = x[:, :, ::self.stride[0], ::self.stride[1]].contiguous(memory_format=torch.channels_last)
        return _C.gemm_bias_act(x, self.weight, self.bias, residual, self.relu)

    def _one_pass(self, x):
        return _C.conv_bias_act(x, self.weight, self.bias_lp, self.stride, self.padding, self.relu)

    def _measure(self, x, two=None, one=None):
        two, one = two or self._two_pass, one or self._one_pass

        def timed(fn):
            fn(x)
            times = []
            for _ in range(5):
                e0, e1 = torch.cuda.Event(enable_timing=True), torch.cuda.Event(enable_timing=True)
                e0.record()
                fn(x)
                e1.record()
                e1.synchronize()
                times.append(e0.elapsed_time(e1) * 1e3)
            return sorted(times)[2]
        t_two = timed(two)
        try:
            t_one = timed(one)
        except RuntimeError:
            t_one = float('inf')
        return (t_one < t_two, t_one, t_two)

    def forward(self, x, residual=None):
        if self.pointwise and _C.gemm_available():
            if tuple(self.stride) != (1, 1):
                if (residual is None and self.strided_ok and _Conv.use_conv_library and x.is_cuda
                        and x.is_contiguous(memory_format=torch.channels_last) and _C.conv_available()):
                    if self._routed(tuple(x.shape), 'act', x, self._copy_then_gemm, self._one_pass):
                        try:
                            return self._one_pass(x)
                        except RuntimeError:
                            self.route[tuple(x.shape)] = (False, float('inf'), 0.0)
                return self._copy_then_gemm(x, residual)
            return _C.gemm_bias_act(x, self.weight, self.bias, residual, self.relu)
        if (residual is None and self.library_ok and _Conv.use_conv_library and x.is_cuda
                and x.is_contiguous(memory_format=torch.channels_last) and _C.conv_available()):
            if self._routed(tuple(x.shape), 'act', x, self._two_pass, self._one_pass):
                try:
                    return self._one_pass(x)
                except RuntimeError:
                    self.route[tuple(x.shape)] = (False, float('inf'), 0.0)
        return self._two_pass(x, residual)

    def _routed(self, key, kind, x, two, one):
        route = self.route.get(key)
        if route is None and _Conv.route_mode != 'auto':
            route = self.route[key] = (_Conv.route_mode == 'library', None, None)
        if route is None and _planning() and not torch.cuda.is_current_stream_capturing():
            route = self.route[key] = self._measure(x, two, one)
            self.learned[kind] = route[0]
        if route is None:
            return self.learned.get(kind, False)
        return route[0]

    def conv_then_pool(self, x):
        y = F.conv2d(x, self.weight, None, self.stride, self.padding, groups=self.groups)
        if y.dtype in (torch.bfloat16, torch.float16) and y.shape[1] % 8 == 0:
            return _C.bias_act_maxpool(y.contiguous(memory_format=torch.channels_last), self.bias, self.relu)
        return F.max_pool2d(_C.bias_act_(y.contiguous(memory_format=torch.channels_last), self.bias, None, self.relu), 3, 2, 1)


class _Block(nn.Module):
    def __init__(self, block, dtype):
        super().__init__()
        if isinstance(block, Bottleneck):
            self.convs = nn.ModuleList([_Conv(block.conv1, block.bn1, True, dtype), _Conv(block.conv2, block.bn2, True, dtype)])
            self.last = _Conv(block.conv3, block.bn3, True, dtype)
        elif isinstance(block, BasicBlock):
            self.convs = nn.ModuleList([_Conv(block.conv1, block.bn1, True, dtype)])
            self.last = _Conv(block.conv2, block.bn2, True, dtype)
        else:
            raise TypeError('unsupported block %r' % type(block))
        self.down = None if block.downsample is None else _Conv(block.downsample[0], block.downsample[1], False, dtype)

    def forward(self, x):
        skip = x if self.down is None else self.down(x)
        y = x
        for c in self.convs:
            y = c(y)
        return self.last(y, skip)


class FusedRetinaNet(nn.Module):
    @staticmethod
    def supports(model):
        if len(model.backbones) != 1:
            return False
        fpn = next(iter(model.backbones.values()))
        net = getattr(fpn, 'features', None)
        if net is None or not all(hasattr(net, n) for n in ('conv1', 'bn1', 'layer1', 'layer2', 'layer3', 'layer4')):
            return False
        if list(getattr(net, 'outputs', [])) != [3, 4, 5]:
            return False
        return all(isinstance(b, (Bottleneck, BasicBlock)) for layer in (net.layer1, net.layer2, net.layer3, net.layer4)
                   for b in layer)

    def __init__(self, model, dtype=torch.bfloat16):
        super().__init__()
        if not self.supports(model):
            raise ValueError('FusedRetinaNet supports a single ResNet-FPN backbone')
        fpn = next(iter(model.backbones.values()))
        net = fpn.features
        self.dtype = dtype
        self.model = [model]
        self.stem = _Conv(net.conv1, net.bn1, True, dtype)
        self.stem_s2d = None
        c1 = net.conv1
        if (tuple(c1.kernel_size), tuple(c1.stride), tuple(c1.padding), c1.in_channels, c1.groups) == ((7, 7), (2, 2), (3, 3), 3, 1) \
                and dtype in (torch.bfloat16, torch.float16):
            w = self.stem.weight.float()
            w4 = stem_space_to_depth_weights(w)
            self.register_buffer('stem_w4', w4.to(dtype).contiguous(memory_format=torch.channels_last))
            self.register_buffer('stem_zero_bias', torch.zeros(w.shape[0], dtype=dtype, device=w.device))
            self.stem_s2d = {}
        self.stem_learned = False
        self.layers = nn.ModuleList([nn.ModuleList([_Block(b, dtype) for b in layer])
                                     for layer in (net.layer1, net.layer2, net.layer3, net.layer4)])
        self.outputs = list(net.outputs)
        self.lateral = nn.ModuleList([_Conv(fpn.lateral3, None, False, dtype), _Conv(fpn.lateral4, None, False, dtype),
                                      _Conv(fpn.lateral5, None, False, dtype)])
        self.smooth = nn.ModuleList([_Conv(fpn.smooth3, None, False, dtype), _Conv(fpn.smooth4, None, False, dtype),
                                     _Conv(fpn.smooth5, None, False, dtype)])
        self.pyramid6 = _Conv(fpn.pyramid6, None, False, dtype)
        self.pyramid7 = _Conv(fpn.pyramid7, None, False, dtype)

        def head(seq):
            convs = [m for m in seq if isinstance(m, nn.Conv2d)]
            return nn.ModuleList([_Conv(c, None, i + 1 < len(convs), dtype) for i, c in enumerate(convs)])

        self.cls_head = head(model.cls_head)
        self.box_head = head(model.box_head)
        self.level_streams = True
        self._streams = None
        self.tower_plan = 0
        self._planned = set()
        self.cls_arena = bool(os.environ.get('ODTK_CLS_ARENA'))
        self._arenas = {}
        self._loaded_geometries = set()
        self._plan_file_seen = False
        self.libraries_taken = None
        self.max_plans = 4
        self._graphs = {}
        self._thresholds = {}
        self.max_graphs = 8

    def _stem_direct(self, x):
        x = x.to(self.dtype).contiguous(memory_format=torch.channels_last)
        return self.stem.conv_then_pool(x)

    def _stem_packed(self, x):
        xs = _C.stem_pack(x, self.dtype)
        y = _C.conv_bias_act(xs, self.stem_w4, self.stem_zero_bias, 1, ((2, 1), (2, 1)), False)
        return _C.bias_act_maxpool(y, self.stem.bias, self.stem.relu)

    def _stem(self, x):
        if (self.stem_s2d is not None and _Conv.use_conv_library and x.is_cuda and x.dim() == 4 and x.shape[1] == 3
                and x.shape[2] % 2 == 0 and x.shape[3] % 2 == 0 and x.dtype in _C._DTYPES and _C.conv_available()
                and (x.is_contiguous() or x.is_contiguous(memory_format=torch.channels_last))):
            key = (tuple(x.shape), x.dtype, x.is_contiguous())
            route = self.stem_s2d.get(key)
            if route is None and _Conv.route_mode != 'auto':
                route = self.stem_s2d[key] = (_Conv.route_mode == 'library', None, None)
            if route is None and _planning() and not torch.cuda.is_current_stream_capturing():
                route = self.stem_s2d[key] = self.stem._measure(x, self._stem_direct, self._stem_packed)
                self.stem_learned = route[0]
            if route[0] if route is not None else self.stem_learned:
                try:
                    return self._stem_packed(x)
                except RuntimeError:
                    self.stem_s2d[key] = (False, float('inf'), 0.0)
        return self._stem_direct(x)

    def features(self, x):
        x = self._stem(x)
        feats = []
        for level, layer in enumerate(self.layers, start=2):
            for block in layer:
                x = block(x)
            if level in self.outputs:
                feats.append(x)
        c3, c4, c5 = feats
        p5 = self.lateral[2](c5)
        p4 = self.lateral[1](c4, self._upsample(p5))
        p3 = self.lateral[0](c3, self._upsample(p4))
        p6 = self.pyramid6(c5)
        p7 = self.pyramid7(F.relu(p6))
        return [self.smooth[0](p3), self.smooth[1](p4), self.smooth[2](p5), p6, p7]

    @staticmethod
    def _upsample(t):
        if (t.is_cuda and t.dtype in _C._DTYPES and t.is_contiguous(memory_format=torch.channels_last)
                and (t.shape[1] * t.element_size()) % 16 == 0):
            return _C.upsample2x(t)
        return F.interpolate(t, scale_factor=2).contiguous(memory_format=torch.channels_last)

    @staticmethod
    def _run(seq, t):
        for c in seq:
            t = c(t)
        return t

    def _towers(self, feats, last_bias, level_streams=None):
        arena = self._cls_arena(feats) if (self.cls_arena and not last_bias and feats[0].is_cuda and not _planning()) else None

        def level(t, i):
            if last_bias:
                return self._run(self.cls_head, t), self._run(self.box_head, t)
            return (self.cls_head[-1].conv_only(self._run(self.cls_head[:-1], t), None if arena is None else arena[i]),
                    self.box_head[-1].conv_only(self._run(self.box_head[:-1], t)))

        if level_streams is None:
            level_streams = self.level_streams
        if not level_streams or not feats[0].is_cuda or len(feats) < 3:
            out = [level(t, i) for i, t in enumerate(feats)]
            return [o[0] for o in out], [o[1] for o in out]
        main = torch.cuda.current_stream(feats[0].device)
        if self._streams is None or self._streams[0].device != feats[0].device:
            self._streams = [torch.cuda.Stream(feats[0].device) for _ in range(3)]
        n = len(feats)
        mine, groups = {0: ([0], [[1], list(range(2, n))]),
                        1: (list(range(2, n)) + [1], [[0]]),
                        2: ([0], [[1], [2], list(range(3, n))])}[self.tower_plan]
        ready = torch.cuda.Event()
        ready.record(main)
        out = [None] * len(feats)
        done = []
        for stream, group in zip(self._streams, groups):
            stream.wait_event(ready)
            with torch.cuda.stream(stream):
                for i in group:
                    out[i] = level(feats[i], i)
                    for t in out[i]:
                        t.record_stream(main)
                e = torch.cuda.Event()
                e.record(stream)
                done.append(e)
        for i in mine:
            out[i] = level(feats[i], i)
        for e in done:
            main.wait_event(e)
        return [o[0] for o in out], [o[1] for o in out]

    def _cls_arena(self, feats):
        channels = self.cls_head[-1].weight.shape[0]
        key = tuple((t.shape[0], t.shape[2], t.shape[3]) for t in feats) + (feats[0].device,)
        hit = self._arenas.get(key)
        if hit is None:
            step = 2 << 20
            elt = torch.empty(0, dtype=self.dtype).element_size()
            sizes = [t.shape[0] * t.shape[2] * t.shape[3] * channels * elt for t in feats]
            total = sum((n + step - 1) // step * step for n in sizes) + step
            buf = torch.empty(total, dtype=torch.uint8, device=feats[0].device)
            off = (-buf.data_ptr()) % step
            views = []
            for t, n in zip(feats, sizes):
                v = buf[off:off + n].view(self.dtype).view(t.shape[0], t.shape[2], t.shape[3], channels).permute(0, 3, 1, 2)
                views.append(v)
                off += (n + step - 1) // step * step
            self._arenas.clear()
            hit = self._arenas[key] = (buf, views)
        return hit[1]

    def heads(self, x):
        with torch.autocast(x.device.type, enabled=False):
            return self._towers(self.features(x), True)

    def heads_without_last_bias(self, x):
        with torch.autocast(x.device.type, enabled=False):
            cls, box = self._towers(self.features(x), False)
        return cls, box, self.cls_head[-1].bias, self.box_head[-1].bias

    @torch.no_grad()
    def replay(self, x):
        m = self.model[0]
        bias = self.cls_head[-1].bias
        key = (tuple(x.shape), x.dtype, x.device, x.is_contiguous(memory_format=torch.channels_last),
               m.threshold, m.top_n, m.nms, m.detections, self.level_streams, self.tower_plan, bias.data_ptr(), bias._version)
        entry = self._graphs.get(key)
        if entry is None:
            static_x = torch.empty_like(x)
            static_x.copy_(x)
            side = torch.cuda.Stream(x.device)
            side.wait_stream(torch.cuda.current_stream(x.device))
            with torch.cuda.stream(side):
                for _ in range(2):
                    self.forward(static_x)
            torch.cuda.current_stream(x.device).wait_stream(side)
            graph = torch.cuda.CUDAGraph()
            with torch.cuda.graph(graph):
                out = self.forward(static_x)
            while len(self._graphs) >= self.max_graphs:
                self._graphs.pop(next(iter(self._graphs)))
            entry = self._graphs[key] = (graph, static_x, out, tuple(self._thresholds.values()))
        graph, static_x, out = entry[:3]
        static_x.copy_(x)
        graph.replay()
        return tuple(o.clone() for o in out)

    def plan(self, x):
        path = os.environ.get('ODTK_CONV_PLAN')
        if path and not self._plan_file_seen:
            self._plan_file_seen = True
            if os.path.isfile(path):
                with open(path) as f:
                    self.load_plan(json.load(f))
        key = (tuple(x.shape), x.device)
        if key in self._planned or not x.is_cuda or not _C.conv_available() or not _Conv.use_conv_library:
            return
        if tuple(x.shape) in self._loaded_geometries:
            self._planned.add(key)
            return
        if len(self._planned) >= self.max_plans:
            return
        if torch.cuda.is_current_stream_capturing():
            return
        with _PLAN_LOCK:
            _TLS.planning = True
            try:
                with torch.autocast(x.device.type, enabled=False):
                    self._towers(self.features(x), False, level_streams=False)
            finally:
                _TLS.planning = False
            self._planned.add(key)
        if path:
            self.save_plan(path)

    def plan_state(self):
        layers, learned = {}, {}
        for name, mod in self.named_modules():
            if isinstance(mod, _Conv):
                if mod.route:
                    layers[name] = {_key_str(k): int(bool(v[0])) for k, v in sorted(mod.route.items(), key=lambda kv: _key_str(kv[0]))}
                if mod.learned:
                    learned[name] = {k: bool(v) for k, v in sorted(mod.learned.items())}
        stem = {}
        for (shape, dtype, contiguous), v in (self.stem_s2d or {}).items():
            stem['%s:%s:%d' % ('x'.join(str(int(d)) for d in shape), str(dtype).replace('torch.', ''), int(contiguous))] = int(bool(v[0]))
        geometries = sorted({tuple(k[0]) for k in self._planned} | set(self._loaded_geometries))
        return {'format': 'odtk-conv-plan-1', 'dtype': str(self.dtype).replace('torch.', ''), 'geometries': [list(g) for g in geometries],
                'layers': layers, 'learned': learned, 'stem': dict(sorted(stem.items())), 'stem_learned': bool(self.stem_learned),
                'libraries': sorted(line for line in _C.library_plans_export().splitlines() if line)}

    def plan_hash(self, state=None):
        state = state or self.plan_state()
        text = json.dumps({k: state[k] for k in ('dtype', 'layers', 'stem', 'libraries')}, sort_keys=True)
        return hashlib.sha256(text.encode()).hexdigest()[:16]

    def load_plan(self, state):
        if state.get('format') != 'odtk-conv-plan-1':
            raise ValueError('not an odtk conv plan: format %r' % (state.get('format'),))
        if state.get('dtype') != str(self.dtype).replace('torch.', ''):
            raise ValueError('the plan was made for %s, this engine runs %s' % (state.get('dtype'), self.dtype))
        mods = {name: mod for name, mod in self.named_modules() if isinstance(mod, _Conv)}
        unknown = sorted(set(state.get('layers', {})) - set(mods))
        if unknown:
            raise ValueError('the plan names layers this engine does not have: %s' % ', '.join(unknown[:4]))
        for name, routes in state.get('layers', {}).items():
            for text, use in routes.items():
                mods[name].route[_str_key(text)] = (bool(use), None, None)
        for name, kinds in state.get('learned', {}).items():
            if name in mods:
                mods[name].learned.update({k: bool(v) for k, v in kinds.items()})
        if self.stem_s2d is not None:
            for text, use in state.get('stem', {}).items():
                shape, dtype, contiguous = text.split(':')
                self.stem_s2d[(tuple(int(v) for v in shape.split('x')), getattr(torch, dtype), bool(int(contiguous)))] = (bool(use), None, None)
            self.stem_learned = bool(state.get('stem_learned', self.stem_learned))
        self._loaded_geometries.update(tuple(g) for g in state.get('geometries', []))
        self.libraries_taken = _C.library_plans_import('\n'.join(state.get('libraries', [])) + '\n')
        return self.libraries_taken

    def save_plan(self, path):
        tmp = '%s.%d.tmp' % (path, os.getpid())
        with open(tmp, 'w') as f:
            json.dump(self.plan_state(), f, indent=1, sort_keys=True)
        os.replace(tmp, path)

    def conv_routes(self):
        routes = {name: dict(mod.route) for name, mod in self.named_modules() if isinstance(mod, _Conv) and mod.route}
        if self.stem_s2d:
            routes['stem (cast + conv1 + pool: space-to-depth form vs direct)'] = {k[0]: v for k, v in self.stem_s2d.items()}
        return routes

    @torch.no_grad()
    def forward(self, x):
        m = self.model[0]
        self.plan(x)
        fold = self.dtype in (torch.bfloat16, torch.float16) and self.cls_head[-1].bias.numel() % 8 == 0
        if fold:
            cls_heads, box_heads, cls_bias, box_bias = self.heads_without_last_bias(x)
        else:
            (cls_heads, box_heads), cls_bias, box_bias = self.heads(x), None, None
        strides = [x.shape[-1] // c.shape[-1] for c in cls_heads]
        for s in strides:
            m.level_anchors(s)
        table = None
        if fold and cls_bias.is_cuda and not os.environ.get('ODTK_NO_THRESHOLD_TABLE'):
            key = (float(m.threshold), cls_bias.data_ptr(), cls_bias._version)
            table = self._thresholds.get(key)
            if table is None and not torch.cuda.is_current_stream_capturing():
                self._thresholds.clear()
                table = self._thresholds[key] = _C.prefilter_thresholds(cls_bias, self.dtype, m.threshold)
        if os.environ.get('ODTK_CHECK_FINITE'):
            for name, heads in (('cls', cls_heads), ('box', box_heads)):
                for i, t in enumerate(heads):
                    if not bool(torch.isfinite(t).all()):
                        raise FloatingPointError('FusedRetinaNet: non-finite values in the %s head tensor of level %d' % (name, i))
        return box_ops.detect(cls_heads, box_heads, strides, m.anchors, m.threshold, m.top_n, m.nms, m.detections,
                              m.rotated_bbox, logits=True, cls_bias=cls_bias, box_bias=box_bias, cls_thresholds=table)
```

Before: 1213 images/s.

## Pack FPN levels P4-P7 into one padded canvas for shared head towers

Packs the smaller pyramid levels (feats[1:]) into a single zero-guttered canvas, so the shared cls/box tower convolutions run as one large conv per layer instead of one small conv per level. The gutters are re-zeroed between tower layers, and the final head conv reads strided views of the canvas. To support those views, a strided-input path is added to the CK conv wrapper. The aim is to cut kernel launch count and the low GPU utilisation of the small-level convs, at the cost of extra compute on gutter pixels plus pack and clear kernels. The path is on by default via ODTK_PYRAMID_CANVAS.

```diff
diff --git a/include/odtk_conv.h b/include/odtk_conv.h
--- a/include/odtk_conv.h
+++ b/include/odtk_conv.h
@@ -15,6 +15,7 @@
                             int c_out, int kernel_h, int kernel_w, int stride_h, int stride_w, int pad_h, int pad_w, int pad_h_end,
                             int pad_w_end, int dtype, int relu, void *stream);
 
+
 const char *odtk_conv_last_plan(void);
 
 size_t odtk_conv_plan_export(char *text, size_t capacity);
diff --git a/include/odtk_conv_strided.h b/include/odtk_conv_strided.h
--- /dev/null
+++ b/include/odtk_conv_strided.h
@@ -0,0 +1,19 @@
+#ifndef ODTK_CONV_STRIDED_H
+#define ODTK_CONV_STRIDED_H
+
+#include "odtk_conv.h"
+
+#ifdef __cplusplus
+extern "C" {
+#endif
+
+int odtk_conv_bias_act_strided(void *y, const void *x, const void *w, const void *bias, int batch_size, int c_in, int height, int width,
+                               int c_out, int kernel_h, int kernel_w, int stride_h, int stride_w, int pad_h, int pad_w, int pad_h_end,
+                               int pad_w_end, long long x_image_stride, long long x_row_stride, long long x_pixel_stride,
+                               long long y_image_stride, long long y_row_stride, long long y_pixel_stride, int dtype, int relu,
+                               void *stream);
+
+#ifdef __cplusplus
+}
+#endif
+#endif
diff --git a/include/odtk_hip.h b/include/odtk_hip.h
--- a/include/odtk_hip.h
+++ b/include/odtk_hip.h
@@ -97,6 +97,11 @@
 
 int odtk_upsample_nearest2x(const void *x, void *out, int batch_size, int height, int width, int channels, int dtype,
                             void *stream);
+
+int odtk_canvas_clear(void *canvas, int batch_size, int height, int width, int channels, int dtype, const int *rects, int n_rects,
+                      void *stream);
+int odtk_canvas_pack(void *canvas, int batch_size, int height, int width, int channels, int dtype, const int *rects,
+                     const void *const *sources, int n_rects, void *stream);
 
 int odtk_stem_pack(const void *x, void *out, int batch_size, int height, int width, int in_dtype, int channels_last, int out_dtype,
                    void *stream);
diff --git a/retinanet-examples_amd/csrc/conv_ck.cpp b/retinanet-examples_amd/csrc/conv_ck.cpp
--- a/retinanet-examples_amd/csrc/conv_ck.cpp
+++ b/retinanet-examples_amd/csrc/conv_ck.cpp
@@ -2,7 +2,9 @@
 
 #include <array>
 #include <cfloat>
+#include <cstdint>
 #include <cstdio>
+#include <cstdlib>
 #include <cstring>
 #include <map>
 #include <memory>
@@ -16,7 +18,7 @@
 #include "ck/tensor_operation/gpu/device/tensor_layout.hpp"
 #include "ck/tensor_operation/gpu/element/element_wise_operation.hpp"
 
-#include "../../include/odtk_conv.h"
+#include "../../include/odtk_conv_strided.h"
 #include "../../include/odtk_hip.h"
 
 namespace {
@@ -36,6 +38,13 @@
   bool operator<(const Problem &o) const {
     return std::tie(n, c, h, w, k, r, s, u, v, ph, pw, ph1, pw1, dtype) <
            std::tie(o.n, o.c, o.h, o.w, o.k, o.r, o.s, o.u, o.v, o.ph, o.pw, o.ph1, o.pw1, o.dtype);
+  }
+};
+
+struct Strides {
+  index_t xn, xh, xw, yn, yh, yw;
+  bool operator<(const Strides &o) const {
+    return std::tie(xn, xh, xw, yn, yh, yw) < std::tie(o.xn, o.xh, o.xw, o.yn, o.yh, o.yw);
   }
 };
 
@@ -53,6 +62,7 @@
 struct Instances {
   std::vector<std::unique_ptr<ConvOp<T>>> ops;
   std::map<Problem, Plan> plans;
+  std::map<std::tuple<Problem, Strides, int>, bool> views;
   Instances() { ops = ck::tensor_operation::device::instance::DeviceOperationInstanceFactory<ConvOp<T>>::GetInstances(); }
 };
 
@@ -63,13 +73,13 @@
 }
 
 template <typename T>
-std::unique_ptr<ck::tensor_operation::device::BaseArgument> make_argument(ConvOp<T> &op, const Problem &p, void *y, const void *x,
-                                                                          const void *w, const void *bias, int relu) {
+std::unique_ptr<ck::tensor_operation::device::BaseArgument> make_argument(ConvOp<T> &op, const Problem &p, const Strides &st, void *y,
+                                                                          const void *x, const void *w, const void *bias, int relu) {
   const index_t G = 1, N = p.n, C = p.c, K = p.k, Hi = p.h, Wi = p.w, Y = p.r, X = p.s;
   const index_t Ho = (Hi + p.ph + p.ph1 - Y) / p.u + 1, Wo = (Wi + p.pw + p.pw1 - X) / p.v + 1;
-  const std::array<index_t, 5> a_len{G, N, C, Hi, Wi}, a_str{C, Hi * Wi * G * C, 1, Wi * G * C, G * C};
+  const std::array<index_t, 5> a_len{G, N, C, Hi, Wi}, a_str{C, st.xn, 1, st.xh, st.xw};
   const std::array<index_t, 5> b_len{G, K, C, Y, X}, b_str{K * Y * X * C, Y * X * C, 1, X * C, C};
-  const std::array<index_t, 5> e_len{G, N, K, Ho, Wo}, e_str{K, Ho * Wo * G * K, 1, Wo * G * K, G * K};
+  const std::array<index_t, 5> e_len{G, N, K, Ho, Wo}, e_str{K, st.yn, 1, st.yh, st.yw};
   const std::array<index_t, 5> d_str{K, 0, 1, 0, 0};
   const std::array<index_t, 2> strides{p.u, p.v}, dilations{1, 1}, pads{p.ph, p.pw}, pads_end{p.ph1, p.pw1};
   return op.MakeArgumentPointer(x, w, std::array<const void *, 1>{bias}, y, a_len, a_str, b_len, b_str,
@@ -85,7 +95,8 @@
 }
 
 template <typename T>
-bool adopt_sibling(Instances<T> &inst, const Problem &p, void *y, const void *x, const void *w, const void *bias, int relu, Plan *out) {
+bool adopt_sibling(Instances<T> &inst, const Problem &p, const Strides &st, void *y, const void *x, const void *w, const void *bias, int relu,
+                   Plan *out) {
   const double pixels = static_cast<double>(p.n) * p.h * p.w;
   const Plan *best = nullptr;
   double best_ratio = 2.0;
@@ -101,7 +112,7 @@
   }
   if (!best) return false;
   auto &op = *inst.ops[best->index];
-  auto arg = make_argument<T>(op, p, y, x, w, bias, relu);
+  auto arg = make_argument<T>(op, p, st, y, x, w, bias, relu);
   if (!op.IsSupportedArgument(arg.get()) || op.GetWorkSpaceSize(arg.get()) != 0) return false;
   *out = *best;
   out->us = 0.0f;
@@ -109,7 +120,8 @@
 }
 
 template <typename T>
-int run(const Problem &p, void *y, const void *x, const void *w, const void *bias, int relu, hipStream_t stream, int force_index) {
+int run(const Problem &p, const Strides &st, void *y, const void *x, const void *w, const void *bias, int relu, hipStream_t stream,
+        int force_index) {
   std::lock_guard<std::mutex> lock(g_mutex);
   Instances<T> &inst = instances<T>();
   Plan plan;
@@ -119,13 +131,13 @@
   if (force_index >= 0) {
     plan = Plan{};
     if (force_index < static_cast<int>(inst.ops.size())) {
-      auto arg = make_argument<T>(*inst.ops[force_index], p, y, x, w, bias, relu);
+      auto arg = make_argument<T>(*inst.ops[force_index], p, st, y, x, w, bias, relu);
       if (inst.ops[force_index]->IsSupportedArgument(arg.get()) && inst.ops[force_index]->GetWorkSpaceSize(arg.get()) == 0)
         plan.index = force_index;
     }
     if (plan.index < 0) return ODTK_ERR_UNSUPPORTED;
     plan.name = inst.ops[plan.index]->GetTypeString();
-  } else if (it == inst.plans.end() && adopt_sibling<T>(inst, p, y, x, w, bias, relu, &plan)) {
+  } else if (it == inst.plans.end() && adopt_sibling<T>(inst, p, st, y, x, w, bias, relu, &plan)) {
     inst.plans[p] = plan;
   } else if (it == inst.plans.end() || (!plan.timed && !capturing && plan.index >= 0)) {
     plan = Plan{};
@@ -141,7 +153,7 @@
     for (size_t i = 0; i < inst.ops.size(); ++i) {
       try {
         auto &op = *inst.ops[i];
-        auto arg = make_argument<T>(op, p, y, x, w, bias, relu);
+        auto arg = make_argument<T>(op, p, st, y, x, w, bias, relu);
         if (!op.IsSupportedArgument(arg.get()) || op.GetWorkSpaceSize(arg.get()) != 0) continue;
         if (capturing) { plan.index = static_cast<int>(i); break; }
         auto invoker = op.MakeInvokerPointer();
@@ -169,7 +181,12 @@
   }
   if (plan.index < 0) return ODTK_ERR_UNSUPPORTED;
   auto &op = *inst.ops[plan.index];
-  auto arg = make_argument<T>(op, p, y, x, w, bias, relu);
+  auto arg = make_argument<T>(op, p, st, y, x, w, bias, relu);
+  const auto view = std::make_tuple(p, st, plan.index);
+  auto seen = inst.views.find(view);
+  if (seen == inst.views.end())
+    seen = inst.views.emplace(view, op.IsSupportedArgument(arg.get()) && op.GetWorkSpaceSize(arg.get()) == 0).first;
+  if (!seen->second) return ODTK_ERR_UNSUPPORTED;
   op.MakeInvokerPointer()->Run(arg.get(), StreamConfig{stream, false});
   char buf[64];
   std::snprintf(buf, sizeof buf, "#%d %.1f us ", plan.index, plan.us);
@@ -207,19 +224,36 @@
 
 extern "C" {
 
-int odtk_conv_bias_act_pads(void *y, const void *x, const void *w, const void *bias, int batch_size, int c_in, int height, int width,
-                            int c_out, int kernel_h, int kernel_w, int stride_h, int stride_w, int pad_h, int pad_w, int pad_h_end,
-                            int pad_w_end, int dtype, int relu, void *stream) {
+int odtk_conv_bias_act_strided(void *y, const void *x, const void *w, const void *bias, int batch_size, int c_in, int height, int width,
+                               int c_out, int kernel_h, int kernel_w, int stride_h, int stride_w, int pad_h, int pad_w, int pad_h_end,
+                               int pad_w_end, long long x_image_stride, long long x_row_stride, long long x_pixel_stride,
+                               long long y_image_stride, long long y_row_stride, long long y_pixel_stride, int dtype, int relu,
+                               void *stream) {
   if (!y || !x || !w || !bias || batch_size <= 0 || c_in <= 0 || c_out <= 0 || height <= 0 || width <= 0 || kernel_h <= 0 ||
       kernel_w <= 0 || stride_h <= 0 || stride_w <= 0 || pad_h < 0 || pad_w < 0 || pad_h_end < 0 || pad_w_end < 0)
     return ODTK_ERR_INVALID;
   if (height + pad_h + pad_h_end < kernel_h || width + pad_w + pad_w_end < kernel_w) return ODTK_ERR_INVALID;
   const Problem p{batch_size, c_in, height, width, c_out, kernel_h, kernel_w, stride_h, stride_w, pad_h, pad_w, pad_h_end, pad_w_end, dtype};
+  const long long out_h = (height + pad_h + pad_h_end - kernel_h) / stride_h + 1, out_w = (width + pad_w + pad_w_end - kernel_w) / stride_w + 1;
+  const long long limit = 0x7fffffffll;
+  if (x_pixel_stride < c_in || x_row_stride < (width - 1) * x_pixel_stride + c_in || x_image_stride < (height - 1) * x_row_stride + (width - 1) * x_pixel_stride + c_in ||
+      y_pixel_stride < c_out || y_row_stride < (out_w - 1) * y_pixel_stride + c_out || y_image_stride < (out_h - 1) * y_row_stride + (out_w - 1) * y_pixel_stride + c_out ||
+      x_image_stride > limit || y_image_stride > limit)
+    return ODTK_ERR_INVALID;
+  const bool x_packed = x_pixel_stride == c_in && x_row_stride == width * x_pixel_stride && x_image_stride == height * x_row_stride;
+  const bool y_packed = y_pixel_stride == c_out && y_row_stride == out_w * y_pixel_stride && y_image_stride == out_h * y_row_stride;
+  if (!x_packed && (((x_pixel_stride | x_row_stride | x_image_stride) & 7) || (reinterpret_cast<uintptr_t>(x) & 15u))) return ODTK_ERR_INVALID;
+  if (!y_packed) {
+    if (((y_pixel_stride | y_row_stride | y_image_stride) & 7) || (reinterpret_cast<uintptr_t>(y) & 15u)) return ODTK_ERR_INVALID;
+    if (y_row_stride != out_w * y_pixel_stride || y_image_stride != out_h * y_row_stride) return ODTK_ERR_UNSUPPORTED;
+  }
+  const Strides st{static_cast<index_t>(x_image_stride), static_cast<index_t>(x_row_stride), static_cast<index_t>(x_pixel_stride),
+                   static_cast<index_t>(y_image_stride), static_cast<index_t>(y_row_stride), static_cast<index_t>(y_pixel_stride)};
   int force = -1;
   if (const char *f = std::getenv("ODTK_CONV_INSTANCE")) force = std::atoi(f);
   try {
-    if (dtype == ODTK_BF16) return run<ck::bhalf_t>(p, y, x, w, bias, relu, static_cast<hipStream_t>(stream), force);
-    if (dtype == ODTK_F16) return run<ck::half_t>(p, y, x, w, bias, relu, static_cast<hipStream_t>(stream), force);
+    if (dtype == ODTK_BF16) return run<ck::bhalf_t>(p, st, y, x, w, bias, relu, static_cast<hipStream_t>(stream), force);
+    if (dtype == ODTK_F16) return run<ck::half_t>(p, st, y, x, w, bias, relu, static_cast<hipStream_t>(stream), force);
   } catch (const std::exception &e) {
     g_last_plan = std::string("exception: ") + e.what();
     return ODTK_ERR_UNSUPPORTED;
@@ -228,6 +262,18 @@
     return ODTK_ERR_UNSUPPORTED;
   }
   return ODTK_ERR_UNSUPPORTED;
+}
+
+int odtk_conv_bias_act_pads(void *y, const void *x, const void *w, const void *bias, int batch_size, int c_in, int height, int width,
+                            int c_out, int kernel_h, int kernel_w, int stride_h, int stride_w, int pad_h, int pad_w, int pad_h_end,
+                            int pad_w_end, int dtype, int relu, void *stream) {
+  if (c_in <= 0 || c_out <= 0 || height <= 0 || width <= 0 || kernel_h <= 0 || kernel_w <= 0 || stride_h <= 0 || stride_w <= 0 ||
+      pad_h < 0 || pad_w < 0 || pad_h_end < 0 || pad_w_end < 0 || height + pad_h + pad_h_end < kernel_h || width + pad_w + pad_w_end < kernel_w)
+    return ODTK_ERR_INVALID;
+  const long long out_h = (height + pad_h + pad_h_end - kernel_h) / stride_h + 1, out_w = (width + pad_w + pad_w_end - kernel_w) / stride_w + 1;
+  return odtk_conv_bias_act_strided(y, x, w, bias, batch_size, c_in, height, width, c_out, kernel_h, kernel_w, stride_h, stride_w, pad_h,
+                                    pad_w, pad_h_end, pad_w_end, 1ll * height * width * c_in, 1ll * width * c_in, c_in,
+                                    out_h * out_w * c_out, out_w * c_out, c_out, dtype, relu, stream);
 }
 
 int odtk_conv_bias_act(void *y, const void *x, const void *w, const void *bias, int batch_size, int c_in, int height, int width,
diff --git a/retinanet-examples_amd/csrc/epilogue.hpp b/retinanet-examples_amd/csrc/epilogue.hpp
--- a/retinanet-examples_amd/csrc/epilogue.hpp
+++ b/retinanet-examples_amd/csrc/epilogue.hpp
@@ -184,6 +184,32 @@
   }
 }
 
+struct CanvasArgs {
+  uint32_t n;
+  uint32_t y0[ODTK_MAX_LEVELS], x0[ODTK_MAX_LEVELS], h[ODTK_MAX_LEVELS], w[ODTK_MAX_LEVELS];
+  const vuint4 *src[ODTK_MAX_LEVELS];
+};
+
+__global__ __launch_bounds__(256) void canvas_fill_kernel(vuint4 *__restrict__ canvas, const CanvasArgs a, uint32_t groups, uint32_t total,
+                                                          const FastDiv by_groups, const FastDiv by_w, const FastDiv by_h) {
+  for (uint32_t i = blockIdx.x * 256u + threadIdx.x; i < total; i += gridDim.x * 256u) {
+    uint32_t g, x, y;
+    uint32_t p = fastdivmod(i, by_groups, &g);
+    p = fastdivmod(p, by_w, &x);
+    const uint32_t b = fastdivmod(p, by_h, &y);
+    bool inside = false;
+#pragma unroll
+    for (uint32_t l = 0; l < ODTK_MAX_LEVELS; ++l) {
+      const uint32_t dy = y - a.y0[l], dx = x - a.x0[l];
+      if (l < a.n && dy < a.h[l] && dx < a.w[l]) {
+        inside = true;
+        if (a.src[l]) canvas[i] = a.src[l][((static_cast<uint64_t>(b) * a.h[l] + dy) * a.w[l] + dx) * groups + g];
+      }
+    }
+    if (!inside) canvas[i] = vuint4{0u, 0u, 0u, 0u};
+  }
+}
+
 template <typename TIn, typename TOut>
 __global__ __launch_bounds__(256) void stem_pack_kernel(const void *x, void *out, uint32_t batch, uint32_t height, uint32_t width,
                                                         uint32_t channels_last, FastDiv by_wo, FastDiv by_howo) {
diff --git a/retinanet-examples_amd/csrc/odtk_hip.hip b/retinanet-examples_amd/csrc/odtk_hip.hip
--- a/retinanet-examples_amd/csrc/odtk_hip.hip
+++ b/retinanet-examples_amd/csrc/odtk_hip.hip
@@ -1065,6 +1065,42 @@
   return ODTK_OK;
 }
 
+int odtk_canvas_pack(void *canvas, int batch_size, int height, int width, int channels, int dtype, const int *rects,
+                     const void *const *sources, int n_rects, void *stream) {
+  if (!canvas || !rects || batch_size <= 0 || height <= 0 || width <= 0 || channels <= 0 || n_rects < 0 || n_rects > ODTK_MAX_LEVELS)
+    return ODTK_ERR_INVALID;
+  if (dtype != ODTK_F32 && dtype != ODTK_BF16 && dtype != ODTK_F16) return ODTK_ERR_UNSUPPORTED;
+  const unsigned long long row_bytes = 1ull * channels * (dtype == ODTK_F32 ? 4 : 2);
+  if (row_bytes % 16) return ODTK_ERR_UNSUPPORTED;
+  if (reinterpret_cast<uintptr_t>(canvas) & 15u) return ODTK_ERR_INVALID;
+  const unsigned long long groups = row_bytes / 16;
+  const unsigned long long total = 1ull * batch_size * height * width * groups;
+  if (total > 0xf0000000ull) return ODTK_ERR_INVALID;
+  odtk::CanvasArgs a{};
+  a.n = static_cast<uint32_t>(n_rects);
+  for (int l = 0; l < n_rects; ++l) {
+    const int y0 = rects[4 * l], x0 = rects[4 * l + 1], h = rects[4 * l + 2], w = rects[4 * l + 3];
+    if (y0 < 0 || x0 < 0 || h <= 0 || w <= 0 || y0 > height - h || x0 > width - w) return ODTK_ERR_INVALID;
+    if (sources && (!sources[l] || (reinterpret_cast<uintptr_t>(sources[l]) & 15u))) return ODTK_ERR_INVALID;
+    a.y0[l] = static_cast<uint32_t>(y0); a.x0[l] = static_cast<uint32_t>(x0);
+    a.h[l] = static_cast<uint32_t>(h); a.w[l] = static_cast<uint32_t>(w);
+    a.src[l] = sources ? static_cast<const odtk::vuint4 *>(sources[l]) : nullptr;
+  }
+  unsigned long long blocks = (total + 256ull * 4 - 1) / (256ull * 4);
+  if (blocks > 256 * 16) blocks = 256 * 16;
+  hipLaunchKernelGGL(odtk::canvas_fill_kernel, dim3(static_cast<unsigned>(blocks)), dim3(256), 0, static_cast<hipStream_t>(stream),
+                     static_cast<odtk::vuint4 *>(canvas), a, static_cast<uint32_t>(groups), static_cast<uint32_t>(total),
+                     odtk::fastdiv_make(static_cast<uint32_t>(groups)), odtk::fastdiv_make(static_cast<uint32_t>(width)),
+                     odtk::fastdiv_make(static_cast<uint32_t>(height)));
+  ODTK_HIP_TRY(hipGetLastError());
+  return ODTK_OK;
+}
+
+int odtk_canvas_clear(void *canvas, int batch_size, int height, int width, int channels, int dtype, const int *rects, int n_rects,
+                      void *stream) {
+  return odtk_canvas_pack(canvas, batch_size, height, width, channels, dtype, rects, nullptr, n_rects, stream);
+}
+
 int odtk_stem_pack(const void *x, void *out, int batch_size, int height, int width, int in_dtype, int channels_last, int out_dtype,
                    void *stream) {
   if (!x || !out || batch_size <= 0 || height <= 0 || width <= 0 || (height & 1) || (width & 1)) return ODTK_ERR_INVALID;
diff --git a/retinanet-examples_amd/odtk/_C.py b/retinanet-examples_amd/odtk/_C.py
--- a/retinanet-examples_amd/odtk/_C.py
+++ b/retinanet-examples_amd/odtk/_C.py
@@ -95,6 +95,9 @@
     'odtk_prefilter_thresholds': (ctypes.c_int, [_vp, ctypes.c_int, ctypes.c_int, ctypes.c_float, _vp, _vp]),
     'odtk_upsample_nearest2x': (ctypes.c_int, [ctypes.c_void_p, ctypes.c_void_p, ctypes.c_int, ctypes.c_int, ctypes.c_int, ctypes.c_int,
                                                ctypes.c_int, ctypes.c_void_p]),
+    'odtk_canvas_clear': (ctypes.c_int, [ctypes.c_void_p] + [ctypes.c_int] * 5 + [ctypes.POINTER(ctypes.c_int), ctypes.c_int, ctypes.c_void_p]),
+    'odtk_canvas_pack': (ctypes.c_int, [ctypes.c_void_p] + [ctypes.c_int] * 5 + [ctypes.POINTER(ctypes.c_int), _vpp, ctypes.c_int,
+                                        ctypes.c_void_p]),
     'odtk_stem_pack': (ctypes.c_int, [ctypes.c_void_p, ctypes.c_void_p, ctypes.c_int, ctypes.c_int, ctypes.c_int, ctypes.c_int,
                                       ctypes.c_int, ctypes.c_int, ctypes.c_void_p]),
     'odtk_preprocess_images': (ctypes.c_int, [ctypes.c_int, ctypes.POINTER(Image), _vp, _sz, _vp, _sz, _vp, _vp, ctypes.c_int, ctypes.c_int,
@@ -685,6 +688,46 @@
     return out
 
 
+def _canvas_args(canvas, rects, what):
+    if not canvas.is_cuda or canvas.dim() != 4 or canvas.dtype not in _DTYPES:
+        raise RuntimeError('%s: canvas must be a 4-d CUDA tensor of float32/bfloat16/float16' % what)
+    n, c, h, w = canvas.shape
+    if not canvas.is_contiguous(memory_format=torch.channels_last) or (c * canvas.element_size()) % 16:
+        raise RuntimeError('%s: canvas must be channels_last with channels * element size a multiple of 16 bytes' % what)
+    if len(rects) > MAX_LEVELS:
+        raise RuntimeError('%s: at most %d rectangles' % (what, MAX_LEVELS))
+    flat = [int(v) for r in rects for v in r]
+    if len(flat) != 4 * len(rects):
+        raise RuntimeError('%s: a rectangle is (y0, x0, height, width)' % what)
+    return n, c, h, w, (ctypes.c_int * max(len(flat), 1))(*flat)
+
+
+def canvas_clear_(canvas, rects):
+    n, c, h, w, arr = _canvas_args(canvas, rects, 'canvas_clear_')
+    with torch.cuda.device(canvas.device):
+        stream = torch.cuda.current_stream(canvas.device).cuda_stream
+        _check(library().odtk_canvas_clear(canvas.data_ptr(), n, h, w, c, _DTYPES[canvas.dtype], arr, len(rects), stream), 'canvas_clear')
+    return canvas
+
+
+def canvas_pack(levels, rects, height, width):
+    first = levels[0]
+    n, c = first.shape[:2]
+    if len(levels) != len(rects):
+        raise RuntimeError('canvas_pack: one rectangle per level')
+    for t, r in zip(levels, rects):
+        if (not t.is_cuda or t.dim() != 4 or t.dtype != first.dtype or t.device != first.device or tuple(t.shape) != (n, c, r[2], r[3])
+                or not (t.is_contiguous(memory_format=torch.channels_last))):
+            raise RuntimeError('canvas_pack: every level must be a channels_last [B, C, h, w] CUDA tensor of one dtype filling its rectangle')
+    canvas = torch.empty((n, c, height, width), dtype=first.dtype, device=first.device, memory_format=torch.channels_last)
+    n, c, h, w, arr = _canvas_args(canvas, rects, 'canvas_pack')
+    with torch.cuda.device(canvas.device):
+        stream = torch.cuda.current_stream(canvas.device).cuda_stream
+        _check(library().odtk_canvas_pack(canvas.data_ptr(), n, h, w, c, _DTYPES[canvas.dtype], arr, _ptrs(list(levels)), len(rects), stream),
+               'canvas_pack')
+    return canvas
+
+
 def stem_pack(x, dtype):
     if not x.is_cuda or x.dim() != 4 or x.shape[1] != 3 or x.dtype not in _DTYPES or dtype not in (torch.bfloat16, torch.float16):
         raise RuntimeError('stem_pack: x must be a [B, 3, H, W] CUDA tensor of float32/bfloat16/float16, dtype bfloat16/float16')
@@ -786,6 +829,9 @@
             lib.odtk_conv_bias_act.argtypes = [ctypes.c_void_p] * 4 + [ctypes.c_int] * 13 + [ctypes.c_void_p]
             lib.odtk_conv_bias_act_pads.restype = ctypes.c_int
             lib.odtk_conv_bias_act_pads.argtypes = [ctypes.c_void_p] * 4 + [ctypes.c_int] * 15 + [ctypes.c_void_p]
+            lib.odtk_conv_bias_act_strided.restype = ctypes.c_int
+            lib.odtk_conv_bias_act_strided.argtypes = ([ctypes.c_void_p] * 4 + [ctypes.c_int] * 13 + [ctypes.c_longlong] * 6 +
+                                                       [ctypes.c_int] * 2 + [ctypes.c_void_p])
             lib.odtk_conv_last_plan.restype = ctypes.c_char_p
             lib.odtk_conv_last_plan.argtypes = []
             lib.odtk_conv_instance_count.restype = ctypes.c_int
@@ -813,8 +859,6 @@
     k, c2, kh, kw = weight.shape
     if c2 != c or weight.dtype != x.dtype or not weight.is_contiguous(memory_format=torch.channels_last):
         raise RuntimeError('conv_bias_act: weight must be [Cout, Cin, kh, kw] of x.dtype, channels_last')
-    if not x.is_contiguous(memory_format=torch.channels_last):
-        raise RuntimeError('conv_bias_act: x must be channels_last')
     if bias.dtype != x.dtype or bias.numel() != k or not bias.is_cuda or not bias.is_contiguous():
         raise RuntimeError('conv_bias_act: bias must be a CUDA vector of length Cout in the dtype of x')
     sh, sw = (stride, stride) if isinstance(stride, int) else stride
@@ -824,14 +868,24 @@
     if out is None:
         y = torch.empty((b, k, ho, wo), dtype=x.dtype, device=x.device, memory_format=torch.channels_last)
     else:
-        if tuple(out.shape) != (b, k, ho, wo) or out.dtype != x.dtype or out.device != x.device or \
-                not out.is_contiguous(memory_format=torch.channels_last):
+        if tuple(out.shape) != (b, k, ho, wo) or out.dtype != x.dtype or out.device != x.device:
             raise RuntimeError('conv_bias_act: out must be a channels_last %s tensor of shape %s' % (x.dtype, (b, k, ho, wo)))
         y = out
+    views = []
+    for t, name in ((x, 'x'), (y, 'out')):
+        sn, sc, srow, spix = t.stride()
+        if t.shape[1] != 1 and sc != 1:
+            raise RuntimeError('conv_bias_act: %s must be channels_last (or a view of a channels_last tensor)' % name)
+        ch, hh, ww = t.shape[1], t.shape[2], t.shape[3]
+        spix = spix if ww > 1 else ch
+        srow = srow if hh > 1 else ww * spix
+        sn = sn if t.shape[0] > 1 else hh * srow
+        views += [sn, srow, spix]
     with torch.cuda.device(x.device):
         stream = torch.cuda.current_stream(x.device).cuda_stream
-        _check(lib.odtk_conv_bias_act_pads(y.data_ptr(), x.data_ptr(), weight.data_ptr(), bias.data_ptr(), b, c, h, w, k, kh, kw,
-                                           sh, sw, ph0, pw0, ph1, pw1, _DTYPES[x.dtype], 1 if relu else 0, stream), 'conv_bias_act')
+        _check(lib.odtk_conv_bias_act_strided(y.data_ptr(), x.data_ptr(), weight.data_ptr(), bias.data_ptr(), b, c, h, w, k, kh, kw,
+                                              sh, sw, ph0, pw0, ph1, pw1, *views, _DTYPES[x.dtype], 1 if relu else 0, stream),
+               'conv_bias_act')
     return y
 
 
diff --git a/retinanet-examples_amd/odtk/fused.py b/retinanet-examples_amd/odtk/fused.py
--- a/retinanet-examples_amd/odtk/fused.py
+++ b/retinanet-examples_amd/odtk/fused.py
@@ -58,6 +58,31 @@
     b, _, h, w = x.shape
     xs = x.view(b, 3, h // 2, 2, w // 2, 2).permute(0, 3, 5, 1, 2, 4).reshape(b, 12, h // 2, w // 2)
     return torch.cat([xs, torch.zeros(b, 4, h // 2, w // 2, dtype=x.dtype, device=x.device)], 1)
+
+
+def pyramid_canvas_layout(shapes, gutter=1):
+    shapes = [(int(h), int(w)) for h, w in shapes]
+    if not shapes or min(min(s) for s in shapes) <= 0 or gutter < 0:
+        raise ValueError('pyramid_canvas_layout: needs positive extents and a gutter >= 0')
+    height = max(h for h, _ in shapes)
+    origins = [(0, 0)]
+    shelf_x = shapes[0][1] + gutter
+    shelf_w, row_y, row_h, cursor = None, 0, 0, shelf_x
+    for h, w in shapes[1:]:
+        if shelf_w is None:
+            shelf_w = w
+        elif cursor + w > shelf_x + shelf_w and row_y + row_h + gutter + h <= height:
+            row_y, row_h, cursor = row_y + row_h + gutter, 0, shelf_x
+        origins.append((row_y, cursor))
+        shelf_w = max(shelf_w, cursor + w - shelf_x)
+        row_h = max(row_h, h)
+        cursor += w + gutter
+    return ((max(y + h for (y, _), (h, _) in zip(origins, shapes)), max(x + w for (_, x), (_, w) in zip(origins, shapes))), origins)
+
+
+def _window(x):
+    return (x.dim() == 4 and x.shape[1] > 1 and x.stride(1) == 1 and x.stride(3) >= x.shape[1]
+            and all(v % 8 == 0 for v in (x.stride(0), x.stride(2), x.stride(3))))
 
 
 class _Conv(nn.Module):
@@ -95,6 +120,28 @@
                     self.route[key] = (False, float('inf'), 0.0)
         y = self._miopen_only(x)
         return y if out is None else out.copy_(y)
+
+    def on_view(self, x, only=False, out=None):
+        if x.is_contiguous(memory_format=torch.channels_last):
+            return self.conv_only(x, out) if only else self(x)
+        if self.library_ok and _Conv.use_conv_library and x.is_cuda and _window(x) and _C.conv_available():
+            if only and self.zero_bias is None:
+                self.zero_bias = torch.zeros_like(self.bias_lp)
+            key = (('only',) + tuple(x.shape)) if only else tuple(x.shape)
+            two, one = (self._miopen_only, self._library_only) if only else (self._two_pass, self._one_pass)
+            if self._routed(key, 'only' if only else 'act', x, two, one):
+                try:
+                    return self._library_only(x, out) if only else self._one_pass(x)
+                except RuntimeError:
+                    pass
+        x = x.contiguous(memory_format=torch.channels_last)
+        return self.conv_only(x, out) if only else self(x)
+
+    def _torch(self, x, residual=None):
+        y = F.conv2d(x, self.weight, None, self.stride, self.padding, groups=self.groups) + self.bias.to(x.dtype).view(1, -1, 1, 1)
+        if residual is not None:
+            y = y + residual
+        return (F.relu(y) if self.relu else y).contiguous(memory_format=torch.channels_last)
 
     def _miopen_only(self, x):
         y = F.conv2d(x, self.weight, None, self.stride, self.padding, groups=self.groups)
@@ -138,6 +185,8 @@
         return (t_one < t_two, t_one, t_two)
 
     def forward(self, x, residual=None):
+        if not x.is_cuda:
+            return self._torch(x, residual)
         if self.pointwise and _C.gemm_available():
             if tuple(self.stride) != (1, 1):
                 if (residual is None and self.strided_ok and _Conv.use_conv_library and x.is_cuda
@@ -170,6 +219,8 @@
         return route[0]
 
     def conv_then_pool(self, x):
+        if not x.is_cuda:
+            return F.max_pool2d(self._torch(x), 3, 2, 1)
         y = F.conv2d(x, self.weight, None, self.stride, self.padding, groups=self.groups)
         if y.dtype in (torch.bfloat16, torch.float16) and y.shape[1] % 8 == 0:
             return _C.bias_act_maxpool(y.contiguous(memory_format=torch.channels_last), self.bias, self.relu)
@@ -247,6 +298,7 @@
         self.cls_head = head(model.cls_head)
         self.box_head = head(model.box_head)
         self.level_streams = True
+        self.pyramid_canvas = os.environ.get('ODTK_PYRAMID_CANVAS', '1') != '0'
         self._streams = None
         self.tower_plan = 0
         self._planned = set()
@@ -316,8 +368,56 @@
             t = c(t)
         return t
 
+    def _canvas_gutter(self, feats):
+        if not self.pyramid_canvas or len(feats) < 3 or not (feats[0].is_cuda or self.pyramid_canvas == 'always'):
+            return None
+        gutter = 0
+        for c in list(self.cls_head[:-1]) + list(self.box_head[:-1]):
+            kh, kw = c.weight.shape[2:]
+            if (tuple(c.stride) != (1, 1) or c.groups != 1 or kh % 2 == 0 or kw % 2 == 0 or tuple(c.padding) != (kh // 2, kw // 2)
+                    or c.weight.shape[0] != c.weight.shape[1]):
+                return None
+            gutter = max(gutter, kh // 2, kw // 2)
+        first = feats[1]
+        if any(t.shape[:2] != first.shape[:2] or t.dtype != first.dtype for t in feats[2:]):
+            return None
+        if first.is_cuda and ((first.shape[1] * first.element_size()) % 16 or len(feats) - 1 > _C.MAX_LEVELS
+                              or not all(t.is_contiguous(memory_format=torch.channels_last) for t in feats[1:])):
+            return None
+        return gutter
+
+    def _canvas_towers(self, feats, gutter, last_bias, arena=None):
+        shapes = [(t.shape[2], t.shape[3]) for t in feats]
+        (height, width), origins = pyramid_canvas_layout(shapes, gutter)
+        rects = [(y, x, h, w) for (y, x), (h, w) in zip(origins, shapes)]
+        if feats[0].is_cuda:
+            canvas = _C.canvas_pack(feats, rects, height, width)
+            mask = None
+        else:
+            first = feats[0]
+            canvas = torch.zeros((first.shape[0], first.shape[1], height, width), dtype=first.dtype).contiguous(memory_format=torch.channels_last)
+            mask = torch.ones((1, 1, height, width), dtype=torch.bool)
+            for t, (y, x, h, w) in zip(feats, rects):
+                canvas[:, :, y:y + h, x:x + w] = t
+                mask[:, :, y:y + h, x:x + w] = False
+        out = []
+        for which, head in enumerate((self.cls_head, self.box_head)):
+            t = canvas
+            for j, c in enumerate(head[:-1]):
+                t = c(t)
+                if gutter and j + 2 < len(head):
+                    t = _C.canvas_clear_(t, rects) if t.is_cuda else t.masked_fill_(mask, 0)
+            last = head[-1]
+            views = [t[:, :, y:y + h, x:x + w] for y, x, h, w in rects]
+            if last_bias:
+                out.append([last.on_view(v) for v in views])
+            else:
+                out.append([last.on_view(v, True, None if (arena is None or which) else arena[i]) for i, v in enumerate(views)])
+        return list(zip(*out))
+
     def _towers(self, feats, last_bias, level_streams=None):
         arena = self._cls_arena(feats) if (self.cls_arena and not last_bias and feats[0].is_cuda and not _planning()) else None
+        out = [None] * len(feats)
 
         def level(t, i):
             if last_bias:
@@ -325,34 +425,45 @@
             return (self.cls_head[-1].conv_only(self._run(self.cls_head[:-1], t), None if arena is None else arena[i]),
                     self.box_head[-1].conv_only(self._run(self.box_head[:-1], t)))
 
+        def unit(i):
+            if i == 'canvas':
+                out[1:] = self._canvas_towers(feats[1:], gutter, last_bias, None if arena is None else arena[1:])
+                return out[1:]
+            out[i] = level(feats[i], i)
+            return [out[i]]
+
+        gutter = self._canvas_gutter(feats)
         if level_streams is None:
             level_streams = self.level_streams
         if not level_streams or not feats[0].is_cuda or len(feats) < 3:
-            out = [level(t, i) for i, t in enumerate(feats)]
+            for i in ([0, 'canvas'] if gutter is not None else range(len(feats))):
+                unit(i)
             return [o[0] for o in out], [o[1] for o in out]
         main = torch.cuda.current_stream(feats[0].device)
         if self._streams is None or self._streams[0].device != feats[0].device:
             self._streams = [torch.cuda.Stream(feats[0].device) for _ in range(3)]
         n = len(feats)
-        mine, groups = {0: ([0], [[1], list(range(2, n))]),
-                        1: (list(range(2, n)) + [1], [[0]]),
-                        2: ([0], [[1], [2], list(range(3, n))])}[self.tower_plan]
+        if gutter is not None:
+            mine, groups = {0: ([0], [['canvas']]), 1: (['canvas'], [[0]]), 2: ([0], [['canvas']])}[self.tower_plan]
+        else:
+            mine, groups = {0: ([0], [[1], list(range(2, n))]),
+                            1: (list(range(2, n)) + [1], [[0]]),
+                            2: ([0], [[1], [2], list(range(3, n))])}[self.tower_plan]
         ready = torch.cuda.Event()
         ready.record(main)
-        out = [None] * len(feats)
         done = []
         for stream, group in zip(self._streams, groups):
             stream.wait_event(ready)
             with torch.cuda.stream(stream):
                 for i in group:
-                    out[i] = level(feats[i], i)
-                    for t in out[i]:
-                        t.record_stream(main)
+                    for pair in unit(i):
+                        for t in pair:
+                            t.record_stream(main)
                 e = torch.cuda.Event()
                 e.record(stream)
                 done.append(e)
         for i in mine:
-            out[i] = level(feats[i], i)
+            unit(i)
         for e in done:
             main.wait_event(e)
         return [o[0] for o in out], [o[1] for o in out]
@@ -391,7 +502,7 @@
         m = self.model[0]
         bias = self.cls_head[-1].bias
         key = (tuple(x.shape), x.dtype, x.device, x.is_contiguous(memory_format=torch.channels_last),
-               m.threshold, m.top_n, m.nms, m.detections, self.level_streams, self.tower_plan, bias.data_ptr(), bias._version)
+               m.threshold, m.top_n, m.nms, m.detections, self.level_streams, self.tower_plan, self.pyramid_canvas, bias.data_ptr(), bias._version)
         entry = self._graphs.get(key)
         if entry is None:
             static_x = torch.empty_like(x)
```

After: 1254 images/s, median of 6. +3.4%, better.
